# PufferAI/PufferLib

Hardware: AMD Instinct MI355X
Metric: env steps/sec end-to-end PPO (rollout+GAE+update), 4096 envs (higher is better)
Workload: dtype f32; 1 GPU; squared d=3 nt=1, 4096 envs/GPU x 128 steps, obs 49->64 f32 rows, MLP 128, 4 minibatches x 4 epochs, bptt 16 (BASELINE configs[1]); global_batch=524288, parallelism=dp1

## Files before the change

include/pufferlib_amd.h:

```cpp
#ifndef PUFFERLIB_AMD_H
#define PUFFERLIB_AMD_H
#include <stddef.h>
#include <stdint.h>

#ifdef __cplusplus
extern "C" {
#endif

typedef void *pfa_stream_t;

int pfa_version(void);
const char *pfa_last_error(void);

int pfa_timing_enable(int mode);
int pfa_timing_select(const char *kernel);
int pfa_timing_stride(int every);
int pfa_timing_reset(void);
int pfa_timing_read(const char *kernel, int64_t *launches_host, double *total_ms_host);

size_t pfa_gae_workspace_bytes(int64_t n);
int pfa_gae_f32(const float *dones, const float *values, const float *rewards, float *advantages,
                float *returns, int64_t n, float gamma, float gae_lambda, void *workspace,
                pfa_stream_t stream);
int pfa_gae_sums_supported(int64_t n, int32_t num_envs, int32_t num_minibatches, int32_t bptt_horizon);
size_t pfa_gae_sums_workspace_bytes(int64_t n, int32_t num_minibatches);
int pfa_gae_sums_f32(const float *dones, const float *values, const float *rewards, float *advantages, float *returns,
                     int64_t n, float gamma, float gae_lambda, int32_t num_envs, int32_t num_minibatches, int32_t bptt_horizon,
                     double *adv_stats, double *ev4, double *zero8, void *workspace, pfa_stream_t stream);
int32_t pfa_gae_halo_rows(float gamma, float gae_lambda);
int pfa_gae_halo_publish(const float *dones, const float *values, const float *rewards, int64_t n, float gamma, float gae_lambda,
                         const double *extra, int32_t n_extra, double *out, int32_t rank, int32_t world, pfa_stream_t stream);
int pfa_gae_halo_unpack(const double *gathered, int32_t rank, int32_t world, int64_t n, float gamma, float gae_lambda, float *dones,
                        float *values, float *rewards, pfa_stream_t stream);
int pfa_gae_halo_f32(const float *dones, const float *values, const float *rewards, float *advantages, float *returns, int64_t n,
                     int32_t halo_len, float gamma, float gae_lambda, int32_t num_envs, int32_t num_minibatches, int32_t bptt_horizon,
                     double *adv_stats, double *ev4, double *zero8, void *workspace, pfa_stream_t stream);
int pfa_gae_shard_pass2(const float *dones, const float *values, const float *rewards, float *advantages,
                        float *returns, int64_t n, int has_next, float gamma, float gae_lambda,
                        const void *workspace, const double *carry_in, pfa_stream_t stream);
int pfa_gae_shard_publish(const float *dones, const float *values, const float *rewards, int64_t n, float gamma, float gae_lambda,
                          void *workspace, const double *extra, int32_t n_extra, double *out, int32_t rank, int32_t world,
                          pfa_stream_t stream);
int pfa_gae_shard_fold(const double *gathered, int32_t rank, int32_t world, int64_t n, float gamma, float gae_lambda, void *workspace,
                       float *dones, float *values, float *rewards, double *carry_out, pfa_stream_t stream);


typedef struct {
    int32_t num_envs;
    int32_t distance_to_target;
    int32_t num_targets;
    int32_t obs_stride;
    int32_t tape_rounds;
} pfa_squared_config;

size_t pfa_squared_state_bytes(const pfa_squared_config *cfg);
int pfa_squared_async_reset(void *state, const pfa_squared_config *cfg, int64_t seed, float *obs,
                            float *rewards, uint8_t *terminals, uint8_t *truncations, uint8_t *masks,
                            pfa_stream_t stream);
int pfa_squared_fill_tape(void *state, const pfa_squared_config *cfg, int32_t rounds, pfa_stream_t stream);
int pfa_squared_send(void *state, const pfa_squared_config *cfg, const int64_t *actions, float *obs,
                     float *rewards, uint8_t *terminals, uint8_t *truncations, uint8_t *masks,
                     pfa_stream_t stream);
int pfa_squared_episode_stats(void *state, const pfa_squared_config *cfg, double *out4, int32_t reset,
                              pfa_stream_t stream);
int pfa_squared_last_infos(void *state, const pfa_squared_config *cfg, uint8_t *finished,
                           double *episode_return, int32_t *episode_length, double *score,
                           pfa_stream_t stream);
int pfa_squared_debug_targets(void *state, const pfa_squared_config *cfg, int32_t *cells, pfa_stream_t stream);
int pfa_squared_debug_stream_pos(void *state, const pfa_squared_config *cfg, uint64_t *pos_device, pfa_stream_t stream);

typedef struct {
    int32_t obs_dim;
    int32_t obs_stride;
    int32_t hidden;
    int32_t num_actions;
    uint32_t heads;
} pfa_mlp_dims;

int64_t pfa_mlp_param_count(const pfa_mlp_dims *dims);

typedef struct {
    uint64_t seed;
    uint64_t step;
} pfa_noise_key;

int pfa_mlp_forward_sample(const float *obs, int64_t rows, const float *params, const pfa_mlp_dims *dims,
                           const float *noise, const pfa_noise_key *key, int64_t row_offset,
                           int64_t *actions, float *logprob, float *entropy, float *value,
                           pfa_stream_t stream);

int pfa_philox_exp_noise(float *out, int64_t steps, int64_t rows, int32_t num_actions, const pfa_noise_key *key,
                         int64_t row_offset, pfa_stream_t stream);

typedef struct {
    float *obs;
    int32_t *actions;
    float *logprobs;
    float *values;
    float *rewards;
    float *dones;
    float *advantages;
    float *returns;
    int32_t horizon_T;
} pfa_experience;

int pfa_rollout_mlp_squared(void *state, const pfa_squared_config *cfg, const float *params,
                            const pfa_mlp_dims *dims, const pfa_experience *exp, const float *noise,
                            const pfa_noise_key *key, int64_t env_offset, float *obs, float *rewards,
                            uint8_t *terminals, uint8_t *truncations, uint8_t *masks, pfa_stream_t stream);

typedef struct pfa_mlp_view {
    const float *w1;
    int32_t ldw1, obs_dim, obs_stride, hidden, num_actions, reserved;
    const float *b1, *w2, *b2, *wv, *bv;
} pfa_mlp_view;
int pfa_mlp_view_supported(const pfa_mlp_view *view);
int pfa_mlp_view_forward_sample(const float *obs, int64_t rows, const pfa_mlp_view *view, const float *noise,
                                const pfa_noise_key *key, int64_t row_offset, int64_t *actions, float *logprob,
                                float *entropy, float *value, pfa_stream_t stream);
int pfa_rollout_mlp_view_squared(void *state, const pfa_squared_config *cfg, const pfa_mlp_view *view, const pfa_experience *exp,
                                 const float *noise, const pfa_noise_key *key, int64_t env_offset, float *obs, float *rewards,
                                 uint8_t *terminals, uint8_t *truncations, uint8_t *masks, pfa_stream_t stream);



size_t pfa_stochastic_state_bytes(int32_t num_envs);
int pfa_stochastic_async_reset(void *state, int32_t num_envs, float *obs, float *rewards, uint8_t *terminals,
                               uint8_t *truncations, uint8_t *masks, pfa_stream_t stream);
int pfa_stochastic_send(void *state, int32_t num_envs, double p, int32_t horizon, const int64_t *actions, float *obs,
                        float *rewards, uint8_t *terminals, uint8_t *truncations, uint8_t *masks, pfa_stream_t stream);
int pfa_stochastic_episode_stats(void *state, int32_t num_envs, double *out4, int32_t reset, pfa_stream_t stream);
int pfa_stochastic_last_infos(void *state, int32_t num_envs, uint8_t *finished, double *episode_return,
                              int32_t *episode_length, double *score, pfa_stream_t stream);
int pfa_rollout_mlp_stochastic(void *state, int32_t num_envs, double p, int32_t horizon, const float *params,
                               const pfa_mlp_dims *dims, const pfa_experience *exp, const float *noise,
                               const pfa_noise_key *key, int64_t env_offset, float *obs, float *rewards,
                               uint8_t *terminals, uint8_t *truncations, uint8_t *masks, pfa_stream_t stream);

typedef struct {
    int32_t num_envs;
    int32_t mem_length;
    int32_t mem_delay;
    int32_t tape_rounds;
} pfa_memory_config;
size_t pfa_memory_state_bytes(const pfa_memory_config *cfg);
int pfa_memory_async_reset(void *state, const pfa_memory_config *cfg, int64_t seed, float *obs, float *rewards,
                           uint8_t *terminals, uint8_t *truncations, uint8_t *masks, pfa_stream_t stream);
int pfa_memory_fill_tape(void *state, const pfa_memory_config *cfg, int32_t rounds, pfa_stream_t stream);
int pfa_memory_send(void *state, const pfa_memory_config *cfg, const int64_t *actions, float *obs, float *rewards,
                    uint8_t *terminals, uint8_t *truncations, uint8_t *masks, pfa_stream_t stream);
int pfa_memory_episode_stats(void *state, const pfa_memory_config *cfg, double *out4, int32_t reset, pfa_stream_t stream);
int pfa_memory_last_infos(void *state, const pfa_memory_config *cfg, uint8_t *finished, double *episode_return,
                          int32_t *episode_length, double *score, pfa_stream_t stream);
int pfa_memory_debug_solutions(void *state, const pfa_memory_config *cfg, uint32_t *bits, int32_t *underrun,
                               pfa_stream_t stream);

size_t pfa_bandit_state_bytes(int32_t num_envs);
int pfa_bandit_async_reset(void *state, int32_t num_envs, float *obs, float *rewards, uint8_t *terminals,
                           uint8_t *truncations, uint8_t *masks, pfa_stream_t stream);
int pfa_bandit_send(void *state, int32_t num_envs, int32_t solution, double reward_scale, const double *noise,
                    const int64_t *actions, float *obs, float *rewards, uint8_t *terminals, uint8_t *truncations,
                    uint8_t *masks, pfa_stream_t stream);
int pfa_bandit_episode_stats(void *state, int32_t num_envs, double *out4, int32_t reset, pfa_stream_t stream);
int pfa_bandit_last_infos(void *state, int32_t num_envs, uint8_t *finished, double *episode_return,
                          int32_t *episode_length, double *score, pfa_stream_t stream);

size_t pfa_multiagent_state_bytes(int32_t num_envs);
int pfa_multiagent_async_reset(void *state, int32_t num_envs, float *obs, float *rewards, uint8_t *terminals,
                               uint8_t *truncations, uint8_t *masks, pfa_stream_t stream);
int pfa_multiagent_send(void *state, int32_t num_envs, const int64_t *actions, float *obs, float *rewards,
                        uint8_t *terminals, uint8_t *truncations, uint8_t *masks, pfa_stream_t stream);
int pfa_multiagent_episode_stats(void *state, int32_t num_envs, double *out4, int32_t reset, pfa_stream_t stream);

typedef struct {
    int32_t num_envs;
    int32_t tape_rounds;
} pfa_spaces_config;
size_t pfa_spaces_state_bytes(const pfa_spaces_config *cfg);
int pfa_spaces_async_reset(void *state, const pfa_spaces_config *cfg, int64_t seed, float *obs, float *rewards,
                           uint8_t *terminals, uint8_t *truncations, uint8_t *masks, pfa_stream_t stream);
int pfa_spaces_fill_tape(void *state, const pfa_spaces_config *cfg, int32_t rounds, pfa_stream_t stream);
int pfa_spaces_send(void *state, const pfa_spaces_config *cfg, const int64_t *actions, float *obs, float *rewards,
                    uint8_t *terminals, uint8_t *truncations, uint8_t *masks, pfa_stream_t stream);
int pfa_spaces_episode_stats(void *state, const pfa_spaces_config *cfg, double *out5, int32_t reset, pfa_stream_t stream);
int pfa_spaces_last_infos(void *state, const pfa_spaces_config *cfg, uint8_t *finished, double *episode_return,
                          int32_t *episode_length, double *score, pfa_stream_t stream);

typedef struct {
    int32_t num_envs;
    int32_t obs_values;
    int32_t obs_stride;
    int32_t num_actions;
    int32_t episode_length;
    int32_t obs_high;
    uint64_t seed;
    int64_t env_offset;
} pfa_synth_config;
size_t pfa_synth_state_bytes(const pfa_synth_config *cfg);
int pfa_synth_async_reset(void *state, const pfa_synth_config *cfg, float *obs, float *rewards, uint8_t *terminals,
                          uint8_t *truncations, uint8_t *masks, pfa_stream_t stream);
int pfa_synth_send(void *state, const pfa_synth_config *cfg, const int64_t *actions, float *obs, float *rewards,
                   uint8_t *terminals, uint8_t *truncations, uint8_t *masks, pfa_stream_t stream);
int pfa_frames_async_reset(void *state, const pfa_synth_config *cfg, uint8_t *obs, float *rewards, uint8_t *terminals,
                           uint8_t *truncations, uint8_t *masks, pfa_stream_t stream);
int pfa_frames_send(void *state, const pfa_synth_config *cfg, const int64_t *actions, uint8_t *obs, float *rewards,
                    uint8_t *terminals, uint8_t *truncations, uint8_t *masks, pfa_stream_t stream);
int pfa_synth_episode_stats(void *state, const pfa_synth_config *cfg, double *out4, int32_t reset, pfa_stream_t stream);
int pfa_synth_last_infos(void *state, const pfa_synth_config *cfg, uint8_t *finished, double *episode_return,
                         int32_t *episode_length, double *score, pfa_stream_t stream);

#define PFA_NAT_MAX_FIELDS 32
typedef enum {
    PFA_NAT_U8 = 0, PFA_NAT_I8 = 1, PFA_NAT_U16 = 2, PFA_NAT_I16 = 3, PFA_NAT_U32 = 4, PFA_NAT_I32 = 5,
    PFA_NAT_U64 = 6, PFA_NAT_I64 = 7, PFA_NAT_F16 = 8, PFA_NAT_F32 = 9, PFA_NAT_F64 = 10
} pfa_nat_dtype;
typedef struct {
    void *out;
    int32_t offset;
    int32_t count;
    int32_t dtype;
    int32_t to_f32;
    int32_t out_stride;
    int32_t reserved;
} pfa_nat_field;
int pfa_nativize_rows(const void *rows, int64_t num_rows, int32_t row_bytes, const pfa_nat_field *fields ,
                      int32_t num_fields, pfa_stream_t stream);

typedef struct {
    float clip_coef, vf_clip_coef, vf_coef, ent_coef;
    int32_t norm_adv, clip_vloss;
    int32_t num_minibatches;
    int32_t bptt_horizon;
} pfa_ppo_hparams;

size_t pfa_ppo_workspace_bytes(const pfa_mlp_dims *dims, int64_t batch_rows, const pfa_ppo_hparams *hp);
int pfa_ppo_adv_stats(const pfa_experience *exp, int64_t batch_rows, const pfa_ppo_hparams *hp,
                      double *stats, void *workspace, pfa_stream_t stream);
int pfa_ppo_mlp_grad(const pfa_experience *exp, int64_t batch_rows, int32_t mb, const float *params,
                     const pfa_mlp_dims *dims, const pfa_ppo_hparams *hp, const double *adv_stats,
                     int64_t global_mb_rows, float *grads, void *workspace, pfa_stream_t stream);
int pfa_ppo_mlp_grad_mfma_per_tile(int32_t obs_dim, int32_t obs_stride, int32_t num_actions);
int pfa_ppo_grid_status(void);
int pfa_ppo_grid_reset(void);
int pfa_ppo_mlp_grad_path(const pfa_mlp_dims *dims, int64_t mb_rows);
int pfa_adam_clip_step(float *params, const float *grads, float *exp_avg, float *exp_avg_sq, int64_t count,
                       float lr, float beta1, float beta2, float eps, int64_t step, float max_grad_norm,
                       float grad_scale, const float *loss_sums, double *losses, double loss_scale,
                       const double *norm_partials, int32_t n_norm_partials, pfa_stream_t stream);

int pfa_ppo_mlp_train(const pfa_experience *exp, int64_t batch_rows, float *params, const pfa_mlp_dims *dims,
                      const pfa_ppo_hparams *hp, const double *adv_stats, float *grads, float *exp_avg,
                      float *exp_avg_sq, int64_t opt_step, float lr, float beta1, float beta2, float eps,
                      float max_grad_norm, int32_t update_epochs, double *losses, void *workspace,
                      int32_t data_parallel, pfa_stream_t stream);
int pfa_ppo_mlp_train_logged(const pfa_experience *exp, int64_t batch_rows, float *params, const pfa_mlp_dims *dims,
                             const pfa_ppo_hparams *hp, const double *adv_stats, float *grads, float *exp_avg,
                             float *exp_avg_sq, int64_t opt_step, float lr, float beta1, float beta2, float eps,
                             float max_grad_norm, int32_t update_epochs, double *losses, void *workspace,
                             int32_t data_parallel, const double *log_ev4, double *log_out10, int32_t *log_packed,
                             pfa_stream_t stream);

int pfa_ppo_wide_supported(const pfa_mlp_view *view);
size_t pfa_ppo_wide_workspace_bytes(const pfa_mlp_view *view);
int pfa_ppo_wide_grad(const pfa_experience *exp, int64_t batch_rows, int32_t mb, const pfa_mlp_view *params, const pfa_mlp_view *grads,
                      float *tail16, const pfa_ppo_hparams *hp, const double *adv_stats, int64_t global_mb_rows, void *workspace,
                      pfa_stream_t stream);

int64_t pfa_lstm_param_count(const pfa_mlp_dims *dims);
size_t pfa_lstm_pack_bytes(void);
int pfa_lstm_pack(const float *params, const pfa_mlp_dims *dims, void *wpack, pfa_stream_t stream);
int pfa_lstm_policy_step(const float *obs, int64_t rows, const float *params, const pfa_mlp_dims *dims,
                         const void *wpack, float *h, float *c, const float *noise, const pfa_noise_key *key,
                         int64_t row_offset, int64_t *actions, float *logprob, float *entropy, float *value,
                         pfa_stream_t stream);
int pfa_rollout_lstm_squared(void *state, const pfa_squared_config *cfg, const float *params,
                             const pfa_mlp_dims *dims, const void *wpack, float *h, float *c,
                             const pfa_experience *exp, const float *noise, const pfa_noise_key *key,
                             int64_t env_offset, float *obs, float *rewards, uint8_t *terminals,
                             uint8_t *truncations, uint8_t *masks, pfa_stream_t stream);
int pfa_rollout_lstm_memory(void *state, const pfa_memory_config *cfg, const float *params, const pfa_mlp_dims *dims,
                            const void *wpack, float *h, float *c, const pfa_experience *exp, const float *noise,
                            const pfa_noise_key *key, int64_t env_offset, float *obs, float *rewards, uint8_t *terminals,
                            uint8_t *truncations, uint8_t *masks, pfa_stream_t stream);
int pfa_rollout_lstm_synth(void *state, const pfa_synth_config *cfg, const float *params, const pfa_mlp_dims *dims,
                           const void *wpack, float *h, float *c, const pfa_experience *exp, const float *noise,
                           const pfa_noise_key *key, int64_t env_offset, float *obs, float *rewards, uint8_t *terminals,
                           uint8_t *truncations, uint8_t *masks, pfa_stream_t stream);
int pfa_lstm_pack_bwd(const float *params, const pfa_mlp_dims *dims, void *wpack_bwd, pfa_stream_t stream);
int pfa_lstm_pack_both(const float *params, const pfa_mlp_dims *dims, void *wpack, void *wpack_bwd, pfa_stream_t stream);
int pfa_lstm_seq_forward(const float *obs_tm, int64_t rows, int32_t steps, const float *params, const pfa_mlp_dims *dims,
                         const void *wpack, float *xe, float *gates_act, float *hs, float *cs, int32_t init_slot, pfa_stream_t stream);
size_t pfa_lstm_seq_backward_workspace_bytes(int64_t rows);
int pfa_lstm_seq_backward(const float *gates_act, const float *cs, const float *xe, const float *dh_heads, int64_t rows,
                          int32_t steps, const void *wpack_bwd, float *dgates, float *dxe, float *gate_bias_grad,
                          float *enc_bias_grad, void *workspace, pfa_stream_t stream);
int pfa_store_step(const pfa_experience *exp, int32_t t, int32_t num_envs, int32_t obs_stride, const float *obs,
                   const float *rewards, const uint8_t *terminals, const int64_t *actions, const float *logprob,
                   const float *value, pfa_stream_t stream);
int pfa_store_rows(const pfa_experience *exp, int32_t rows, int32_t num_slots, int32_t obs_stride, const float *obs,
                   const float *rewards, const uint8_t *dones, const int64_t *actions, const float *logprob,
                   const float *value, const int32_t *env_ids, const uint8_t *mask, int32_t *counters,
                   int32_t *stored_dropped, pfa_stream_t stream);
int pfa_store_rows_bytes(const pfa_experience *exp, int32_t rows, int32_t num_slots, int32_t row_bytes, const uint8_t *obs,
                         const float *rewards, const uint8_t *dones, const int64_t *actions, const float *logprob,
                         const float *value, const int32_t *env_ids, const uint8_t *mask, int32_t *counters,
                         int32_t *stored_dropped, pfa_stream_t stream);
int pfa_gather_obs_time_major(const pfa_experience *exp, int64_t batch_rows, int32_t mb, const pfa_ppo_hparams *hp,
                              int32_t obs_stride, float *out, pfa_stream_t stream);
size_t pfa_lstm_heads_loss_workspace_bytes(void);
int pfa_lstm_heads_loss(const float *h, const pfa_experience *exp, int64_t batch_rows, int32_t mb, const float *params,
                        const pfa_mlp_dims *dims, const pfa_ppo_hparams *hp, const double *adv_stats,
                        int64_t global_mb_rows, float *dout, float *dh, float *loss_sums8, float *head_bias_grad16,
                        void *workspace, pfa_stream_t stream);
size_t pfa_gemm_tn_workspace_bytes(int32_t mo, int32_t no, int64_t k);
int pfa_gemm_tn_f32(const float *a, int64_t lda, const float *b, int64_t ldb, float *c, int64_t ldc, int32_t mo,
                    int32_t no, int64_t k, void *workspace, pfa_stream_t stream);
size_t pfa_gemm_tn2_workspace_bytes(int32_t mo, int64_t k);
typedef struct pfa_reduce_job {
    int32_t kind, splits, mo, no;
    const float *partial;
    float *c;
    int64_t ldc;
    float *c2;
    int64_t ldc2;
    int32_t nb, reserved;
} pfa_reduce_job;
int pfa_gemm_tn_partial_f32(const float *a, int64_t lda, const float *b, int64_t ldb, int32_t mo, int32_t no, int64_t k, void *workspace,
                            pfa_reduce_job *job, pfa_stream_t stream);
int pfa_gemm_tn2_partial_f32(const float *a, int64_t lda, const float *b0, int64_t ldb0, const float *b1, int64_t ldb1, int32_t mo, int64_t k,
                             void *workspace, pfa_reduce_job *job, pfa_stream_t stream);
int pfa_reduce_multi(const pfa_reduce_job *jobs, int32_t njobs, pfa_stream_t stream);
int pfa_gemm_tn2_f32(const float *a, int64_t lda, const float *b0, int64_t ldb0, const float *b1, int64_t ldb1, float *c0, int64_t ldc0,
                     float *c1, int64_t ldc1, int32_t mo, int64_t k, void *workspace, pfa_stream_t stream);
int pfa_lstm_finish_grads(float *grads, const pfa_mlp_dims *dims, const float *g16, const float *bsum16, pfa_stream_t stream);
int pfa_sumsq_partials(const float *grads, int64_t count, double *partials, int32_t n, pfa_stream_t stream);

int pfa_dist_unique_id(uint8_t *id128_host);
int pfa_dist_init(const uint8_t *id128_host, int32_t rank, int32_t world);
int pfa_dist_finalize(void);
int pfa_dist_all_reduce_f32(float *buf, int64_t count, pfa_stream_t stream);
int pfa_dist_all_reduce_f64(double *buf, int64_t count, pfa_stream_t stream);
int pfa_dist_info(int64_t *out8);

typedef struct {
    int32_t mode;
    int32_t reserved;
    const void *ptr;
    int64_t lda;
    int32_t IC, IH, IW, OC, OH, OW, KH, KW, S;
    int32_t sc, sy, sx, frame_bytes;
} pfa_igemm_operand;
int pfa_igemm_rows(const pfa_igemm_operand *a, int64_t M, int32_t K, const float *B, int32_t ldb, int32_t N, float *C, int32_t ldc,
                   int32_t epilogue, const float *bias, const float *mask, int32_t ldmask, pfa_stream_t stream);
int pfa_igemm_set_products(int32_t mode);
int pfa_igemm_get_products(void);
size_t pfa_igemm_weights_workspace_bytes(int64_t M, int32_t K, int32_t N);
int pfa_igemm_weights(const pfa_igemm_operand *a, int64_t M, int32_t K, const float *D, int32_t ldd, int32_t N, float *out,
                      int32_t perm, int32_t accumulate, float *bias_out, void *workspace, pfa_stream_t stream);
size_t pfa_colsum_workspace_bytes(int32_t N);
int pfa_colsum(const float *D, int64_t M, int32_t N, int32_t ldd, float *out, int32_t accumulate, void *workspace, pfa_stream_t stream);
int pfa_cnn_pack_conv(const float *w, const pfa_igemm_operand *geom, int32_t u8_order, float *fwd, float *dx, pfa_stream_t stream);
int pfa_igemm_rows_add(const pfa_igemm_operand *a, int64_t M, int32_t K, const float *B, int32_t ldb, int32_t N, float *C, int32_t ldc,
                       int32_t epilogue, const float *bias, const float *mask, int32_t ldmask, const float *addend, int32_t ldadd,
                       pfa_stream_t stream);
int pfa_cnn_pack_conv_same(const float *w, const pfa_igemm_operand *geom, int32_t u8, float *fwd, int32_t ldf, float *dx, pfa_stream_t stream);
int pfa_maxpool3s2_forward(const float *in, int64_t frames, int32_t H, int32_t W, int32_t channels, float *out, pfa_stream_t stream);
int pfa_maxpool3s2_backward(const float *in, const float *out, const float *dout, int64_t frames, int32_t H, int32_t W, int32_t channels,
                            float *din, pfa_stream_t stream);
int pfa_cnn_transpose(const float *w, int32_t N, int32_t K, float *out, pfa_stream_t stream);
int pfa_cnn_pack_fc(const float *w, int32_t N, int32_t channels, int32_t hw, float *perm_out, float *t_out, pfa_stream_t stream);
int pfa_cnn_heads_sample(const float *h, int64_t rows, const float *actor_w, const float *actor_b, const float *value_w,
                         const float *value_b, int32_t num_actions, const float *noise, const pfa_noise_key *key, int64_t row_offset,
                         int64_t *actions, float *logprob, float *entropy, float *value, pfa_stream_t stream);
int pfa_cnn_heads_sample_w(const float *h, int32_t hidden, int64_t rows, const float *actor_w, const float *actor_b, const float *value_w,
                           const float *value_b, int32_t num_actions, const float *noise, const pfa_noise_key *key, int64_t row_offset,
                           int64_t *actions, float *logprob, float *entropy, float *value, pfa_stream_t stream);
size_t pfa_cnn_heads_loss_workspace_bytes(void);
int pfa_cnn_heads_loss(const float *h, const pfa_experience *exp, int64_t batch_rows, int32_t mb, int64_t q0, int64_t rows,
                       const float *actor_w, const float *actor_b, const float *value_w, const float *value_b, int32_t num_actions,
                       const pfa_ppo_hparams *hp, const double *adv_stats, int64_t global_mb_rows, float *dout, float *dh,
                       float *loss_pairs16, int32_t accumulate, void *workspace, pfa_stream_t stream);
int pfa_cnn_heads_loss_w(const float *h, int32_t hidden, const pfa_experience *exp, int64_t batch_rows, int32_t mb, int64_t q0, int64_t rows,
                         const float *actor_w, const float *actor_b, const float *value_w, const float *value_b, int32_t num_actions,
                         const pfa_ppo_hparams *hp, const double *adv_stats, int64_t global_mb_rows, float *dout, float *dh,
                         float *loss_pairs16, int32_t accumulate, void *workspace, pfa_stream_t stream);
int pfa_cnn_gather_frames(const uint8_t *frames, int64_t frame_bytes, int64_t batch_rows, int32_t mb, const pfa_ppo_hparams *hp,
                          int64_t q0, int64_t rows, uint8_t *out, pfa_stream_t stream);

int pfa_heads_rows_sample(const float *out, int32_t ld, int64_t rows, int32_t num_actions, uint32_t heads, const float *noise,
                          const pfa_noise_key *key, int64_t row_offset, int64_t *actions, float *logprob, float *entropy,
                          float *value, pfa_stream_t stream);
int pfa_heads_rows_eval(const float *out, int32_t ld, int64_t rows, int32_t num_actions, uint32_t heads, const int64_t *actions,
                        float *logprob, float *entropy, float *value, pfa_stream_t stream);
size_t pfa_heads_rows_loss_workspace_bytes(int64_t rows);
int pfa_heads_rows_loss(const float *out, int32_t ld, const pfa_experience *exp, int64_t batch_rows, int32_t mb, int64_t q0,
                        int64_t rows, int32_t time_major_rows, int32_t num_actions, uint32_t heads, const pfa_ppo_hparams *hp,
                        const double *adv_stats, int64_t global_mb_rows, float *dout, int32_t ldd, int32_t num_out,
                        float *loss_pairs16, int32_t accumulate, void *workspace, pfa_stream_t stream);
int pfa_lstm_cell_forward(float *gates, const float *c_prev, float *c_out, float *h_out, int32_t ldh, float *h_out2, int32_t ldh2,
                          int64_t rows, int32_t hidden, pfa_stream_t stream);
int pfa_lstm_cell_backward(const float *dh_a, int32_t lda, const float *dh_b, int32_t ldb, float *dc, const float *gates_act,
                           const float *c_prev, const float *c, float *dgates, int64_t rows, int32_t hidden, pfa_stream_t stream);
int pfa_rows_perm(const float *src, int32_t lds_, float *dst, int32_t ldd, const float *act, int32_t lda, int64_t rows, int32_t cols,
                  int32_t segments, int32_t steps, int32_t to_time_major, pfa_stream_t stream);

int pfa_p2p_alloc(int64_t cap_bytes, int32_t world, uint8_t *handle64_host);
int pfa_p2p_open(const uint8_t *handles_host, int32_t rank, int32_t world);
int pfa_p2p_close(void);
int pfa_p2p_status(void);
int64_t pfa_p2p_seq(void);
int pfa_p2p_reset(int64_t base);
int pfa_p2p_debug_set_status(int value);
int pfa_p2p_all_reduce_f32(float *buf, int64_t count, pfa_stream_t stream);
int pfa_p2p_all_reduce_f64(double *buf, int64_t count, pfa_stream_t stream);
int pfa_p2p_ll_all_reduce_f32(float *buf, int64_t count, pfa_stream_t stream);
int64_t pfa_p2p_ll_calls(void);
int pfa_p2p_wait_stats(int64_t *out4_host, int reset);
int pfa_p2p_enable(int on);

int pfa_train_log_sums(const pfa_experience *exp, int64_t batch_rows, int32_t num_envs, const double *losses,
                       double *out10, void *workspace, pfa_stream_t stream);

int pfa_train_ev_sums(const pfa_experience *exp, int64_t batch_rows, int32_t num_envs, double *out4, void *workspace,
                      pfa_stream_t stream);
int pfa_train_log_pack(const double *losses, const double *ev4, double *out10, pfa_stream_t stream);

#ifdef __cplusplus
}
#endif
#endif
```

pufferlib_amd/_lib.py:

```python
import ctypes as C
import os
import subprocess

from .exceptions import ExtensionError

HERE = os.path.dirname(os.path.abspath(__file__))
REPO = os.path.dirname(HERE)
CSRC = os.path.join(HERE, 'csrc')
LIB_DIR = os.path.join(HERE, '_lib')
LIB_PATH = os.path.join(LIB_DIR, 'libpufferlib_amd.so')
SOURCES = ['common.cpp', 'dist.cpp', 'p2p.hip', 'gae.hip', 'squared.hip', 'rollout.hip', 'ppo_update.hip', 'lstm.hip', 'gemm.hip', 'lstm_fused.hip', 'lstm_seq.hip', 'stochastic.hip', 'memory.hip', 'bandit.hip', 'multiagent.hip', 'spaces.hip', 'synthetic.hip', 'nativize.hip', 'igemm.hip', 'cnn_heads.hip', 'general.hip', 'ppo_wide.hip']
HEADERS = sorted(f for f in os.listdir(CSRC) if f.endswith('.hpp')) + [os.path.join('..', '..', 'include', 'pufferlib_amd.h')]


def _stale():
    if not os.path.exists(LIB_PATH):
        return True
    t = os.path.getmtime(LIB_PATH)
    deps = [os.path.join(CSRC, f) for f in SOURCES + HEADERS]
    return any(os.path.exists(d) and os.path.getmtime(d) > t for d in deps)


def source_hash():
    import hashlib
    h = hashlib.sha256()
    for f in SOURCES + HEADERS:
        with open(os.path.join(CSRC, f), 'rb') as fh:
            h.update(fh.read())
    return h.hexdigest()[:16]


def build(force=False, verbose=False):
    if not force and not _stale():
        return LIB_PATH
    os.makedirs(LIB_DIR, exist_ok=True)
    hipcc = os.environ.get('HIPCC', '/opt/rocm/bin/hipcc')
    objs = []
    procs = []
    import shlex
    extra = shlex.split(os.environ.get('PFA_HIPCC_FLAGS', ''))
    for src in SOURCES:
        obj = os.path.join(LIB_DIR, os.path.splitext(src)[0] + '.o')
        objs.append(obj)
        cmd = [hipcc, '--offload-arch=gfx950', '-O3', '-std=c++17', '-fPIC'] + extra + ['-x', 'hip', '-c',
               os.path.join(CSRC, src), '-o', obj]
        if verbose:
            print(' '.join(cmd))
        procs.append((src, subprocess.Popen(cmd, stdout=subprocess.PIPE, stderr=subprocess.STDOUT)))
    for src, p in procs:
        out, _ = p.communicate()
        if p.returncode != 0:
            raise ExtensionError(f'hipcc failed on {src}:\n{out.decode()}')
    cmd = [hipcc, '--offload-arch=gfx950', '-shared', '-fPIC', '-o', LIB_PATH] + objs + ['-ldl']
    r = subprocess.run(cmd, stdout=subprocess.PIPE, stderr=subprocess.STDOUT)
    if r.returncode != 0:
        raise ExtensionError(f'link failed:\n{r.stdout.decode()}')
    return LIB_PATH


class SquaredConfig(C.Structure):
    _fields_ = [('num_envs', C.c_int32), ('distance_to_target', C.c_int32), ('num_targets', C.c_int32),
                ('obs_stride', C.c_int32), ('tape_rounds', C.c_int32)]


NAT_MAX_FIELDS = 32


class NatField(C.Structure):
    _fields_ = [('out', C.c_void_p), ('offset', C.c_int32), ('count', C.c_int32), ('dtype', C.c_int32), ('to_f32', C.c_int32),
                ('out_stride', C.c_int32), ('reserved', C.c_int32)]


class MemoryConfig(C.Structure):
    _fields_ = [('num_envs', C.c_int32), ('mem_length', C.c_int32), ('mem_delay', C.c_int32), ('tape_rounds', C.c_int32)]


class SpacesConfig(C.Structure):
    _fields_ = [('num_envs', C.c_int32), ('tape_rounds', C.c_int32)]


class SynthConfig(C.Structure):
    _fields_ = [('num_envs', C.c_int32), ('obs_values', C.c_int32), ('obs_stride', C.c_int32), ('num_actions', C.c_int32),
                ('episode_length', C.c_int32), ('obs_high', C.c_int32), ('seed', C.c_uint64), ('env_offset', C.c_int64)]


class IgemmOperand(C.Structure):
    _fields_ = [('mode', C.c_int32), ('reserved', C.c_int32), ('ptr', C.c_void_p), ('lda', C.c_int64), ('IC', C.c_int32), ('IH', C.c_int32),
                ('IW', C.c_int32), ('OC', C.c_int32), ('OH', C.c_int32), ('OW', C.c_int32), ('KH', C.c_int32), ('KW', C.c_int32), ('S', C.c_int32),
                ('sc', C.c_int32), ('sy', C.c_int32), ('sx', C.c_int32), ('frame_bytes', C.c_int32)]


class MlpDims(C.Structure):
    _fields_ = [('obs_dim', C.c_int32), ('obs_stride', C.c_int32), ('hidden', C.c_int32), ('num_actions', C.c_int32),
                ('heads', C.c_uint32)]


class MlpView(C.Structure):
    _fields_ = [('w1', C.c_void_p), ('ldw1', C.c_int32), ('obs_dim', C.c_int32), ('obs_stride', C.c_int32), ('hidden', C.c_int32),
                ('num_actions', C.c_int32), ('reserved', C.c_int32), ('b1', C.c_void_p), ('w2', C.c_void_p), ('b2', C.c_void_p),
                ('wv', C.c_void_p), ('bv', C.c_void_p)]


class NoiseKey(C.Structure):
    _fields_ = [('seed', C.c_uint64), ('step', C.c_uint64)]


class Experience(C.Structure):
    _fields_ = [('obs', C.c_void_p), ('actions', C.c_void_p), ('logprobs', C.c_void_p), ('values', C.c_void_p),
                ('rewards', C.c_void_p), ('dones', C.c_void_p), ('advantages', C.c_void_p), ('returns', C.c_void_p),
                ('horizon_T', C.c_int32)]


class ReduceJob(C.Structure):
    _fields_ = [('kind', C.c_int32), ('splits', C.c_int32), ('mo', C.c_int32), ('no', C.c_int32), ('partial', C.c_void_p), ('c', C.c_void_p),
                ('ldc', C.c_int64), ('c2', C.c_void_p), ('ldc2', C.c_int64), ('nb', C.c_int32), ('reserved', C.c_int32)]


class PpoHparams(C.Structure):
    _fields_ = [('clip_coef', C.c_float), ('vf_clip_coef', C.c_float), ('vf_coef', C.c_float), ('ent_coef', C.c_float),
                ('norm_adv', C.c_int32), ('clip_vloss', C.c_int32), ('num_minibatches', C.c_int32),
                ('bptt_horizon', C.c_int32)]


P = C.c_void_p
_SIGNATURES = {
    'pfa_version': (C.c_int, []),
    'pfa_last_error': (C.c_char_p, []),
    'pfa_timing_enable': (C.c_int, [C.c_int]),
    'pfa_timing_select': (C.c_int, [C.c_char_p]),
    'pfa_timing_stride': (C.c_int, [C.c_int]),
    'pfa_timing_reset': (C.c_int, []),
    'pfa_timing_read': (C.c_int, [C.c_char_p, C.POINTER(C.c_int64), C.POINTER(C.c_double)]),
    'pfa_gae_workspace_bytes': (C.c_size_t, [C.c_int64]),
    'pfa_gae_f32': (C.c_int, [P, P, P, P, P, C.c_int64, C.c_float, C.c_float, P, P]),
    'pfa_gae_sums_supported': (C.c_int, [C.c_int64, C.c_int32, C.c_int32, C.c_int32]),
    'pfa_gae_sums_workspace_bytes': (C.c_size_t, [C.c_int64, C.c_int32]),
    'pfa_gae_sums_f32': (C.c_int, [P, P, P, P, P, C.c_int64, C.c_float, C.c_float, C.c_int32, C.c_int32, C.c_int32, P, P, P, P, P]),
    'pfa_gae_halo_rows': (C.c_int32, [C.c_float, C.c_float]),
    'pfa_gae_halo_publish': (C.c_int, [P, P, P, C.c_int64, C.c_float, C.c_float, P, C.c_int32, P, C.c_int32, C.c_int32, P]),
    'pfa_gae_halo_unpack': (C.c_int, [P, C.c_int32, C.c_int32, C.c_int64, C.c_float, C.c_float, P, P, P, P]),
    'pfa_gae_halo_f32': (C.c_int, [P, P, P, P, P, C.c_int64, C.c_int32, C.c_float, C.c_float, C.c_int32, C.c_int32, C.c_int32, P, P, P, P, P]),
    'pfa_gae_shard_pass2': (C.c_int, [P, P, P, P, P, C.c_int64, C.c_int, C.c_float, C.c_float, P, P, P]),
    'pfa_gae_shard_publish': (C.c_int, [P, P, P, C.c_int64, C.c_float, C.c_float, P, P, C.c_int32, P, C.c_int32, C.c_int32, P]),
    'pfa_gae_shard_fold': (C.c_int, [P, C.c_int32, C.c_int32, C.c_int64, C.c_float, C.c_float, P, P, P, P, P, P]),
    'pfa_train_ev_sums': (C.c_int, [C.POINTER(Experience), C.c_int64, C.c_int32, P, P, P]),
    'pfa_train_log_pack': (C.c_int, [P, P, P, P]),
    'pfa_squared_state_bytes': (C.c_size_t, [C.POINTER(SquaredConfig)]),
    'pfa_squared_async_reset': (C.c_int, [P, C.POINTER(SquaredConfig), C.c_int64, P, P, P, P, P, P]),
    'pfa_squared_fill_tape': (C.c_int, [P, C.POINTER(SquaredConfig), C.c_int32, P]),
    'pfa_squared_send': (C.c_int, [P, C.POINTER(SquaredConfig), P, P, P, P, P, P, P]),
    'pfa_squared_episode_stats': (C.c_int, [P, C.POINTER(SquaredConfig), P, C.c_int32, P]),
    'pfa_squared_last_infos': (C.c_int, [P, C.POINTER(SquaredConfig), P, P, P, P, P]),
    'pfa_squared_debug_targets': (C.c_int, [P, C.POINTER(SquaredConfig), P, P]),
    'pfa_squared_debug_stream_pos': (C.c_int, [P, C.POINTER(SquaredConfig), P, P]),
    'pfa_mlp_param_count': (C.c_int64, [C.POINTER(MlpDims)]),
    'pfa_mlp_forward_sample': (C.c_int, [P, C.c_int64, P, C.POINTER(MlpDims), P, C.POINTER(NoiseKey), C.c_int64,
                                         P, P, P, P, P]),
    'pfa_philox_exp_noise': (C.c_int, [P, C.c_int64, C.c_int64, C.c_int32, C.POINTER(NoiseKey), C.c_int64, P]),
    'pfa_rollout_mlp_squared': (C.c_int, [P, C.POINTER(SquaredConfig), P, C.POINTER(MlpDims), C.POINTER(Experience),
                                          P, C.POINTER(NoiseKey), C.c_int64, P, P, P, P, P, P]),
    'pfa_mlp_view_supported': (C.c_int, [C.POINTER(MlpView)]),
    'pfa_ppo_wide_supported': (C.c_int, [C.POINTER(MlpView)]),
    'pfa_ppo_wide_workspace_bytes': (C.c_size_t, [C.POINTER(MlpView)]),
    'pfa_ppo_wide_grad': (C.c_int, [C.POINTER(Experience), C.c_int64, C.c_int32, C.POINTER(MlpView), C.POINTER(MlpView), P, C.POINTER(PpoHparams), P,
                                    C.c_int64, P, P]),
    'pfa_mlp_view_forward_sample': (C.c_int, [P, C.c_int64, C.POINTER(MlpView), P, C.POINTER(NoiseKey), C.c_int64, P, P, P, P, P]),
    'pfa_rollout_mlp_view_squared': (C.c_int, [P, C.POINTER(SquaredConfig), C.POINTER(MlpView), C.POINTER(Experience), P, C.POINTER(NoiseKey),
                                               C.c_int64, P, P, P, P, P, P]),
    'pfa_stochastic_state_bytes': (C.c_size_t, [C.c_int32]),
    'pfa_stochastic_async_reset': (C.c_int, [P, C.c_int32, P, P, P, P, P, P]),
    'pfa_stochastic_send': (C.c_int, [P, C.c_int32, C.c_double, C.c_int32, P, P, P, P, P, P, P]),
    'pfa_stochastic_episode_stats': (C.c_int, [P, C.c_int32, P, C.c_int32, P]),
    'pfa_stochastic_last_infos': (C.c_int, [P, C.c_int32, P, P, P, P, P]),
    'pfa_rollout_mlp_stochastic': (C.c_int, [P, C.c_int32, C.c_double, C.c_int32, P, C.POINTER(MlpDims), C.POINTER(Experience),
                                             P, C.POINTER(NoiseKey), C.c_int64, P, P, P, P, P, P]),
    'pfa_memory_state_bytes': (C.c_size_t, [C.POINTER(MemoryConfig)]),
    'pfa_memory_async_reset': (C.c_int, [P, C.POINTER(MemoryConfig), C.c_int64, P, P, P, P, P, P]),
    'pfa_memory_fill_tape': (C.c_int, [P, C.POINTER(MemoryConfig), C.c_int32, P]),
    'pfa_memory_send': (C.c_int, [P, C.POINTER(MemoryConfig), P, P, P, P, P, P, P]),
    'pfa_memory_episode_stats': (C.c_int, [P, C.POINTER(MemoryConfig), P, C.c_int32, P]),
    'pfa_memory_last_infos': (C.c_int, [P, C.POINTER(MemoryConfig), P, P, P, P, P]),
    'pfa_memory_debug_solutions': (C.c_int, [P, C.POINTER(MemoryConfig), P, P, P]),
    'pfa_bandit_state_bytes': (C.c_size_t, [C.c_int32]),
    'pfa_bandit_async_reset': (C.c_int, [P, C.c_int32, P, P, P, P, P, P]),
    'pfa_bandit_send': (C.c_int, [P, C.c_int32, C.c_int32, C.c_double, P, P, P, P, P, P, P, P]),
    'pfa_bandit_episode_stats': (C.c_int, [P, C.c_int32, P, C.c_int32, P]),
    'pfa_bandit_last_infos': (C.c_int, [P, C.c_int32, P, P, P, P, P]),
    'pfa_multiagent_state_bytes': (C.c_size_t, [C.c_int32]),
    'pfa_multiagent_async_reset': (C.c_int, [P, C.c_int32, P, P, P, P, P, P]),
    'pfa_multiagent_send': (C.c_int, [P, C.c_int32, P, P, P, P, P, P, P]),
    'pfa_spaces_state_bytes': (C.c_size_t, [C.POINTER(SpacesConfig)]),
    'pfa_spaces_async_reset': (C.c_int, [P, C.POINTER(SpacesConfig), C.c_int64, P, P, P, P, P, P]),
    'pfa_spaces_fill_tape': (C.c_int, [P, C.POINTER(SpacesConfig), C.c_int32, P]),
    'pfa_spaces_send': (C.c_int, [P, C.POINTER(SpacesConfig), P, P, P, P, P, P, P]),
    'pfa_spaces_episode_stats': (C.c_int, [P, C.POINTER(SpacesConfig), P, C.c_int32, P]),
    'pfa_spaces_last_infos': (C.c_int, [P, C.POINTER(SpacesConfig), P, P, P, P, P]),
    'pfa_synth_state_bytes': (C.c_size_t, [C.POINTER(SynthConfig)]),
    'pfa_synth_async_reset': (C.c_int, [P, C.POINTER(SynthConfig), P, P, P, P, P, P]),
    'pfa_synth_send': (C.c_int, [P, C.POINTER(SynthConfig), P, P, P, P, P, P, P]),
    'pfa_frames_async_reset': (C.c_int, [P, C.POINTER(SynthConfig), P, P, P, P, P, P]),
    'pfa_frames_send': (C.c_int, [P, C.POINTER(SynthConfig), P, P, P, P, P, P, P]),
    'pfa_synth_episode_stats': (C.c_int, [P, C.POINTER(SynthConfig), P, C.c_int32, P]),
    'pfa_synth_last_infos': (C.c_int, [P, C.POINTER(SynthConfig), P, P, P, P, P]),
    'pfa_multiagent_episode_stats': (C.c_int, [P, C.c_int32, P, C.c_int32, P]),
    'pfa_nativize_rows': (C.c_int, [P, C.c_int64, C.c_int32, P, C.c_int32, P]),
    'pfa_ppo_workspace_bytes': (C.c_size_t, [C.POINTER(MlpDims), C.c_int64, C.POINTER(PpoHparams)]),
    'pfa_ppo_adv_stats': (C.c_int, [C.POINTER(Experience), C.c_int64, C.POINTER(PpoHparams), P, P, P]),
    'pfa_ppo_mlp_grad': (C.c_int, [C.POINTER(Experience), C.c_int64, C.c_int32, P, C.POINTER(MlpDims),
                                   C.POINTER(PpoHparams), P, C.c_int64, P, P, P]),
    'pfa_ppo_mlp_train': (C.c_int, [C.POINTER(Experience), C.c_int64, P, C.POINTER(MlpDims), C.POINTER(PpoHparams), P, P, P, P,
                                    C.c_int64, C.c_float, C.c_float, C.c_float, C.c_float, C.c_float, C.c_int32, P, P,
                                    C.c_int32, P]),
    'pfa_ppo_mlp_train_logged': (C.c_int, [C.POINTER(Experience), C.c_int64, P, C.POINTER(MlpDims), C.POINTER(PpoHparams), P, P, P, P,
                                           C.c_int64, C.c_float, C.c_float, C.c_float, C.c_float, C.c_float, C.c_int32, P, P,
                                           C.c_int32, P, P, C.POINTER(C.c_int32), P]),
    'pfa_store_step': (C.c_int, [C.POINTER(Experience), C.c_int32, C.c_int32, C.c_int32, P, P, P, P, P, P, P]),
    'pfa_store_rows': (C.c_int, [C.POINTER(Experience), C.c_int32, C.c_int32, C.c_int32, P, P, P, P, P, P, P, P, P, P, P]),
    'pfa_store_rows_bytes': (C.c_int, [C.POINTER(Experience), C.c_int32, C.c_int32, C.c_int32, P, P, P, P, P, P, P, P, P, P, P]),
    'pfa_gather_obs_time_major': (C.c_int, [C.POINTER(Experience), C.c_int64, C.c_int32, C.POINTER(PpoHparams), C.c_int32, P, P]),
    'pfa_lstm_heads_loss_workspace_bytes': (C.c_size_t, []),
    'pfa_lstm_heads_loss': (C.c_int, [P, C.POINTER(Experience), C.c_int64, C.c_int32, P, C.POINTER(MlpDims),
                                      C.POINTER(PpoHparams), P, C.c_int64, P, P, P, P, P, P]),
    'pfa_lstm_param_count': (C.c_int64, [C.POINTER(MlpDims)]),
    'pfa_lstm_pack_bytes': (C.c_size_t, []),
    'pfa_lstm_pack': (C.c_int, [P, C.POINTER(MlpDims), P, P]),
    'pfa_lstm_policy_step': (C.c_int, [P, C.c_int64, P, C.POINTER(MlpDims), P, P, P, P, C.POINTER(NoiseKey), C.c_int64,
                                       P, P, P, P, P]),
    'pfa_rollout_lstm_squared': (C.c_int, [P, C.POINTER(SquaredConfig), P, C.POINTER(MlpDims), P, P, P, C.POINTER(Experience),
                                           P, C.POINTER(NoiseKey), C.c_int64, P, P, P, P, P, P]),
    'pfa_rollout_lstm_memory': (C.c_int, [P, C.POINTER(MemoryConfig), P, C.POINTER(MlpDims), P, P, P, C.POINTER(Experience),
                                           P, C.POINTER(NoiseKey), C.c_int64, P, P, P, P, P, P]),
    'pfa_rollout_lstm_synth': (C.c_int, [P, C.POINTER(SynthConfig), P, C.POINTER(MlpDims), P, P, P, C.POINTER(Experience),
                                           P, C.POINTER(NoiseKey), C.c_int64, P, P, P, P, P, P]),
    'pfa_lstm_pack_bwd': (C.c_int, [P, C.POINTER(MlpDims), P, P]),
    'pfa_lstm_seq_forward': (C.c_int, [P, C.c_int64, C.c_int32, P, C.POINTER(MlpDims), P, P, P, P, P, C.c_int32, P]),
    'pfa_lstm_pack_both': (C.c_int, [P, C.POINTER(MlpDims), P, P, P]),
    'pfa_lstm_seq_backward_workspace_bytes': (C.c_size_t, [C.c_int64]),
    'pfa_lstm_seq_backward': (C.c_int, [P, P, P, P, C.c_int64, C.c_int32, P, P, P, P, P, P, P]),
    'pfa_gemm_tn_workspace_bytes': (C.c_size_t, [C.c_int32, C.c_int32, C.c_int64]),
    'pfa_gemm_tn_f32': (C.c_int, [P, C.c_int64, P, C.c_int64, P, C.c_int64, C.c_int32, C.c_int32, C.c_int64, P, P]),
    'pfa_gemm_tn2_workspace_bytes': (C.c_size_t, [C.c_int32, C.c_int64]),
    'pfa_gemm_tn_partial_f32': (C.c_int, [P, C.c_int64, P, C.c_int64, C.c_int32, C.c_int32, C.c_int64, P, C.POINTER(ReduceJob), P]),
    'pfa_gemm_tn2_partial_f32': (C.c_int, [P, C.c_int64, P, C.c_int64, P, C.c_int64, C.c_int32, C.c_int64, P, C.POINTER(ReduceJob), P]),
    'pfa_reduce_multi': (C.c_int, [C.POINTER(ReduceJob), C.c_int32, P]),
    'pfa_gemm_tn2_f32': (C.c_int, [P, C.c_int64, P, C.c_int64, P, C.c_int64, P, C.c_int64, P, C.c_int64, C.c_int32, C.c_int64, P, P]),
    'pfa_lstm_finish_grads': (C.c_int, [P, C.POINTER(MlpDims), P, P, P]),
    'pfa_sumsq_partials': (C.c_int, [P, C.c_int64, P, C.c_int32, P]),
    'pfa_dist_unique_id': (C.c_int, [P]),
    'pfa_dist_init': (C.c_int, [P, C.c_int32, C.c_int32]),
    'pfa_dist_finalize': (C.c_int, []),
    'pfa_dist_all_reduce_f32': (C.c_int, [P, C.c_int64, P]),
    'pfa_dist_all_reduce_f64': (C.c_int, [P, C.c_int64, P]),
    'pfa_dist_info': (C.c_int, [P]),
    'pfa_ppo_mlp_grad_mfma_per_tile': (C.c_int, [C.c_int32, C.c_int32, C.c_int32]),
    'pfa_ppo_mlp_grad_path': (C.c_int, [C.POINTER(MlpDims), C.c_int64]),
    'pfa_heads_rows_sample': (C.c_int, [P, C.c_int32, C.c_int64, C.c_int32, C.c_uint32, P, C.POINTER(NoiseKey), C.c_int64, P, P, P, P, P]),
    'pfa_heads_rows_eval': (C.c_int, [P, C.c_int32, C.c_int64, C.c_int32, C.c_uint32, P, P, P, P, P]),
    'pfa_heads_rows_loss_workspace_bytes': (C.c_size_t, [C.c_int64]),
    'pfa_heads_rows_loss': (C.c_int, [P, C.c_int32, C.POINTER(Experience), C.c_int64, C.c_int32, C.c_int64, C.c_int64, C.c_int32, C.c_int32,
                                      C.c_uint32, C.POINTER(PpoHparams), P, C.c_int64, P, C.c_int32, C.c_int32, P, C.c_int32, P, P]),
    'pfa_lstm_cell_forward': (C.c_int, [P, P, P, P, C.c_int32, P, C.c_int32, C.c_int64, C.c_int32, P]),
    'pfa_lstm_cell_backward': (C.c_int, [P, C.c_int32, P, C.c_int32, P, P, P, P, P, C.c_int64, C.c_int32, P]),
    'pfa_rows_perm': (C.c_int, [P, C.c_int32, P, C.c_int32, P, C.c_int32, C.c_int64, C.c_int32, C.c_int32, C.c_int32, C.c_int32, P]),
    'pfa_igemm_set_products': (C.c_int, [C.c_int32]),
    'pfa_igemm_get_products': (C.c_int, []),
    'pfa_igemm_rows': (C.c_int, [C.POINTER(IgemmOperand), C.c_int64, C.c_int32, P, C.c_int32, C.c_int32, P, C.c_int32, C.c_int32, P, P, C.c_int32, P]),
    'pfa_igemm_weights_workspace_bytes': (C.c_size_t, [C.c_int64, C.c_int32, C.c_int32]),
    'pfa_igemm_weights': (C.c_int, [C.POINTER(IgemmOperand), C.c_int64, C.c_int32, P, C.c_int32, C.c_int32, P, C.c_int32, C.c_int32, P, P, P]),
    'pfa_colsum_workspace_bytes': (C.c_size_t, [C.c_int32]),
    'pfa_colsum': (C.c_int, [P, C.c_int64, C.c_int32, C.c_int32, P, C.c_int32, P, P]),
    'pfa_cnn_pack_conv': (C.c_int, [P, C.POINTER(IgemmOperand), C.c_int32, P, P, P]),
    'pfa_igemm_rows_add': (C.c_int, [C.POINTER(IgemmOperand), C.c_int64, C.c_int32, P, C.c_int32, C.c_int32, P, C.c_int32, C.c_int32, P, P, C.c_int32, P,
                                     C.c_int32, P]),
    'pfa_cnn_pack_conv_same': (C.c_int, [P, C.POINTER(IgemmOperand), C.c_int32, P, C.c_int32, P, P]),
    'pfa_maxpool3s2_forward': (C.c_int, [P, C.c_int64, C.c_int32, C.c_int32, C.c_int32, P, P]),
    'pfa_maxpool3s2_backward': (C.c_int, [P, P, P, C.c_int64, C.c_int32, C.c_int32, C.c_int32, P, P]),
    'pfa_cnn_transpose': (C.c_int, [P, C.c_int32, C.c_int32, P, P]),
    'pfa_cnn_pack_fc': (C.c_int, [P, C.c_int32, C.c_int32, C.c_int32, P, P, P]),
    'pfa_cnn_heads_sample': (C.c_int, [P, C.c_int64, P, P, P, P, C.c_int32, P, C.POINTER(NoiseKey), C.c_int64, P, P, P, P, P]),
    'pfa_cnn_heads_sample_w': (C.c_int, [P, C.c_int32, C.c_int64, P, P, P, P, C.c_int32, P, C.POINTER(NoiseKey), C.c_int64, P, P, P, P, P]),
    'pfa_cnn_heads_loss_w': (C.c_int, [P, C.c_int32, C.POINTER(Experience), C.c_int64, C.c_int32, C.c_int64, C.c_int64, P, P, P, P, C.c_int32,
                                       C.POINTER(PpoHparams), P, C.c_int64, P, P, P, C.c_int32, P, P]),
    'pfa_cnn_heads_loss_workspace_bytes': (C.c_size_t, []),
    'pfa_cnn_heads_loss': (C.c_int, [P, C.POINTER(Experience), C.c_int64, C.c_int32, C.c_int64, C.c_int64, P, P, P, P, C.c_int32,
                                     C.POINTER(PpoHparams), P, C.c_int64, P, P, P, C.c_int32, P, P]),
    'pfa_cnn_gather_frames': (C.c_int, [P, C.c_int64, C.c_int64, C.c_int32, C.POINTER(PpoHparams), C.c_int64, C.c_int64, P, P]),
    'pfa_p2p_alloc': (C.c_int, [C.c_int64, C.c_int32, P]),
    'pfa_p2p_open': (C.c_int, [P, C.c_int32, C.c_int32]),
    'pfa_p2p_close': (C.c_int, []),
    'pfa_p2p_status': (C.c_int, []),
    'pfa_ppo_grid_status': (C.c_int, []),
    'pfa_ppo_grid_reset': (C.c_int, []),
    'pfa_p2p_seq': (C.c_int64, []),
    'pfa_p2p_reset': (C.c_int, [C.c_int64]),
    'pfa_p2p_debug_set_status': (C.c_int, [C.c_int]),
    'pfa_p2p_all_reduce_f32': (C.c_int, [P, C.c_int64, P]),
    'pfa_p2p_all_reduce_f64': (C.c_int, [P, C.c_int64, P]),
    'pfa_p2p_ll_all_reduce_f32': (C.c_int, [P, C.c_int64, P]),
    'pfa_p2p_ll_calls': (C.c_int64, []),
    'pfa_p2p_wait_stats': (C.c_int, [P, C.c_int]),
    'pfa_p2p_enable': (C.c_int, [C.c_int]),
    'pfa_train_log_sums': (C.c_int, [C.POINTER(Experience), C.c_int64, C.c_int32, P, P, P, P]),
    'pfa_adam_clip_step': (C.c_int, [P, P, P, P, C.c_int64, C.c_float, C.c_float, C.c_float, C.c_float, C.c_int64,
                                     C.c_float, C.c_float, P, P, C.c_double, P, C.c_int32, P]),
}

_lib = None


def lib():
    global _lib
    if _lib is not None:
        return _lib
    if not os.path.exists(LIB_PATH):
        raise ExtensionError(
            f'{LIB_PATH} is missing: run `python -c "import __graft_entry__ as g; g.build()"` '
            '(hipcc --offload-arch=gfx950).  pufferlib_amd has no CPU fallback.')
    import torch
    try:
        L = C.CDLL(LIB_PATH)
    except OSError as e:
        raise ExtensionError(f'cannot load {LIB_PATH}: {e}') from e
    for name, (res, args) in _SIGNATURES.items():
        try:
            f = getattr(L, name)
        except AttributeError as e:
            raise ExtensionError(f'{LIB_PATH} does not export {name}') from e
        f.restype = res
        f.argtypes = args
    _lib = L
    form = os.environ.get('PFA_MATRIX_PRODUCTS', 'fp32')
    if form not in ('fp32', 'bf16x6'):
        raise ExtensionError(f"PFA_MATRIX_PRODUCTS={form!r}: expected 'fp32' or 'bf16x6'")
    if form == 'bf16x6':
        check(L.pfa_igemm_set_products(1), 'PFA_MATRIX_PRODUCTS')
    return L


def check(rc, what=''):
    if rc != 0:
        msg = lib().pfa_last_error().decode(errors='replace')
        raise ExtensionError(f'{what} failed ({rc}): {msg}')


def ptr(t):
    return None if t is None else C.c_void_p(t.data_ptr())


def stream_handle():
    import torch
    return C.c_void_p(torch.cuda.current_stream().cuda_stream)


def require_gpu():
    import torch
    if not torch.cuda.is_available():
        raise ExtensionError('pufferlib_amd needs a ROCm GPU (torch.cuda.is_available() is False); '
                             'there is no CPU fallback')
```

pufferlib_amd/csrc/ppo_tile.hpp:

```cpp
#pragma once
#include <cmath>

#ifndef PFA_LOSS_EXP_REPAIR_ALL
#define PFA_LOSS_EXP_REPAIR_ALL 0
#endif

#include "common.hpp"
#include "mlp_tile.hpp"

namespace pfa {

constexpr int kNumStats = 8;

struct RowMap {
    int mb, nmb, horizon;
    __device__ __forceinline__ long long flat(long long q) const {
        const long long k = q / horizon, h = q - k * horizon;
        return ((long long)mb + k * nmb) * horizon + h;
    }
    __device__ __forceinline__ unsigned row32(unsigned q) const {
        const unsigned k = q / (unsigned)horizon, h = q - k * (unsigned)horizon;
        return ((unsigned)mb + k * (unsigned)nmb) * (unsigned)horizon + h;
    }
    __device__ __forceinline__ unsigned tile_first(unsigned tile) const {
        return row32(__builtin_amdgcn_readfirstlane(tile) * 16u);
    }
    __device__ __forceinline__ unsigned tile_row(unsigned tile, unsigned first, int r, bool aligned) const {
        return aligned ? first + (unsigned)r : row32(tile * 16u + (unsigned)r);
    }
};

__device__ __forceinline__ void wave_lds_fence() {
    __builtin_amdgcn_fence(__ATOMIC_RELEASE, "wavefront");
    __builtin_amdgcn_wave_barrier();
}

template <bool SWAP>
__device__ __forceinline__ float gsum(float x) {
    if constexpr (SWAP) {
        auto p = __builtin_amdgcn_permlane16_swap(__float_as_uint(x), __float_as_uint(x), false, false);
        const float s = __uint_as_float(p[0]) + __uint_as_float(p[1]);
        auto q = __builtin_amdgcn_permlane32_swap(__float_as_uint(s), __float_as_uint(s), false, false);
        return __uint_as_float(q[0]) + __uint_as_float(q[1]);
    } else {
        x += __shfl_xor(x, 16, 64);
        x += __shfl_xor(x, 32, 64);
        return x;
    }
}
template <bool SWAP>
__device__ __forceinline__ float gmax(float x) {
    if constexpr (SWAP) {
        auto p = __builtin_amdgcn_permlane16_swap(__float_as_uint(x), __float_as_uint(x), false, false);
        const float s = fmaxf(__uint_as_float(p[0]), __uint_as_float(p[1]));
        auto q = __builtin_amdgcn_permlane32_swap(__float_as_uint(s), __float_as_uint(s), false, false);
        return fmaxf(__uint_as_float(q[0]), __uint_as_float(q[1]));
    } else {
        x = fmaxf(x, __shfl_xor(x, 16, 64));
        x = fmaxf(x, __shfl_xor(x, 32, 64));
        return x;
    }
}

__device__ __forceinline__ float loss_exp(float x) {
    const float kL = 1.44269502162933349609375f, kLl = 1.92596298909109e-8f;
    const float t = x * kL;
    const float e = fmaf(x, kLl, fmaf(x, kL, -t));
    const float r = __builtin_amdgcn_exp2f(t);
    return fmaf(r, e * 0.693147182464599609375f, r);
}
__device__ __forceinline__ float loss_exp_softmax(float x) {
#if PFA_LOSS_EXP_REPAIR_ALL
    return loss_exp(x);
#else
    return __builtin_amdgcn_exp2f(x * 1.44269502162933349609375f);
#endif
}
__device__ __forceinline__ float loss_log(float x) {
    const float l2 = __builtin_amdgcn_logf(x);
    return fmaf(l2, 0.693147182464599609375f, l2 * -1.904654323148236e-9f);
}

struct RowScalars {
    int action;
    float old_logprob, old_value, adv, ret, weight;
};

struct LossOut {
    f32x4 dout;
    float pg, v_loss, ent, neg_logratio, kl, clipped;
};

template <bool MH, bool SWAP = false, bool PERM = false>
__device__ __forceinline__ LossOut ppo_loss_tile(const f32x4 &out, const RowScalars &rs, int a, uint32_t heads, int g,
                                                 const pfa_ppo_hparams &hp, float adv_mean, float adv_rden, float inv_rows) {
    float nl[4], p[4], hent[4], ent = 0.0f, new_logprob = 0.0f, new_value = 0.0f;
    bool chosen[4];
    if constexpr (MH) {
#pragma unroll
        for (int r = 0; r < 4; ++r) {
            nl[r] = p[r] = hent[r] = 0.0f;
            chosen[r] = false;
            if (4 * g + r == a) new_value = out[r];
        }
        int start = 0;
        for (int h = 0; h < 8; ++h) {
            const int sz = (int)((heads >> (4 * h)) & 15u);
            if (sz == 0) break;
            bool mem[4];
            float lmax = -INFINITY;
#pragma unroll
            for (int r = 0; r < 4; ++r) {
                const int o = 4 * g + r;
                mem[r] = o >= start && o < start + sz;
                if (mem[r]) lmax = fmaxf(lmax, out[r]);
            }
            lmax = fmaxf(lmax, __shfl_xor(lmax, 16, 64));
            lmax = fmaxf(lmax, __shfl_xor(lmax, 32, 64));
            float ev[4], se = 0.0f;
#pragma unroll
            for (int r = 0; r < 4; ++r) {
                ev[r] = mem[r] ? loss_exp(out[r] - lmax) : 0.0f;
                se += ev[r];
            }
            se += __shfl_xor(se, 16, 64);
            se += __shfl_xor(se, 32, 64);
            const float lse = lmax + loss_log(se), inv_se = __builtin_amdgcn_rcpf(se);
            const int act = start + (int)(((uint32_t)rs.action >> (4 * h)) & 15u);
            float he = 0.0f;
#pragma unroll
            for (int r = 0; r < 4; ++r)
                if (mem[r]) {
                    nl[r] = out[r] - lse;
                    p[r] = ev[r] * inv_se;
                    he -= nl[r] * p[r];
                    chosen[r] = 4 * g + r == act;
                    if (chosen[r]) new_logprob += nl[r];
                }
            he += __shfl_xor(he, 16, 64);
            he += __shfl_xor(he, 32, 64);
#pragma unroll
            for (int r = 0; r < 4; ++r)
                if (mem[r]) hent[r] = he;
            ent += he;
            start += sz;
        }
        new_logprob += __shfl_xor(new_logprob, 16, 64);
        new_logprob += __shfl_xor(new_logprob, 32, 64);
        new_value += __shfl_xor(new_value, 16, 64);
        new_value += __shfl_xor(new_value, 32, 64);
    } else {
    static_assert(!(MH && PERM), "the permuted layout is the single-head form");
    constexpr int NR = PERM ? 3 : 4;
    const int o0 = PERM ? 3 * g : 4 * g;
#pragma unroll
    for (int r = NR; r < 4; ++r) {
        nl[r] = p[r] = 0.0f;
        chosen[r] = false;
    }
    float lmax = -INFINITY;
#pragma unroll
    for (int r = 0; r < NR; ++r)
        if (o0 + r < a) lmax = fmaxf(lmax, out[r]);
    lmax = gmax<SWAP>(lmax);
    float ev[4], se = 0.0f;
#pragma unroll
    for (int r = 0; r < NR; ++r) {
        ev[r] = o0 + r < a ? loss_exp_softmax(out[r] - lmax) : 0.0f;
        se += ev[r];
    }
    se = gsum<SWAP>(se);
    const float lse = lmax + loss_log(se);
    const float inv_se = __builtin_amdgcn_rcpf(se);
#pragma unroll
    for (int r = 0; r < NR; ++r) {
        const int o = o0 + r;
        nl[r] = out[r] - lse;
        p[r] = ev[r] * inv_se;
        if (o < a) ent -= nl[r] * p[r];
        chosen[r] = o == rs.action;
        if (chosen[r]) new_logprob = nl[r];
        if (o == a) new_value = out[r];
    }
    ent = gsum<SWAP>(ent);
    new_logprob = gsum<SWAP>(new_logprob);
    new_value = gsum<SWAP>(new_value);
#pragma unroll
    for (int r = 0; r < 4; ++r) hent[r] = ent;
    }

    const float logratio = new_logprob - rs.old_logprob;
    const float ratio = loss_exp(logratio);
    const float adv = hp.norm_adv ? (rs.adv - adv_mean) * adv_rden : rs.adv;
    const float lo = 1.0f - hp.clip_coef, hi = 1.0f + hp.clip_coef;
    const float pg1 = -adv * ratio;
    const float pg2 = -adv * fminf(fmaxf(ratio, lo), hi);
    const bool inside = ratio >= lo && ratio <= hi;
    float dpg_dratio;
    if (pg1 > pg2) dpg_dratio = -adv;
    else if (pg1 < pg2) dpg_dratio = inside ? -adv : 0.0f;
    else dpg_dratio = inside ? -adv : -0.5f * adv;
    const float scale = inv_rows * rs.weight;
    const float g_lp = dpg_dratio * ratio * scale;

    float v_loss, dv;
    if (hp.clip_vloss) {
        const float du = new_value - rs.ret;
        const float vl_u = du * du;
        const float delta = new_value - rs.old_value;
        const float v_clipped = rs.old_value + fminf(fmaxf(delta, -hp.vf_clip_coef), hp.vf_clip_coef);
        const float dc = v_clipped - rs.ret;
        const float vl_c = dc * dc;
        const bool vin = delta >= -hp.vf_clip_coef && delta <= hp.vf_clip_coef;
        v_loss = 0.5f * fmaxf(vl_u, vl_c);
        const float gu = 2.0f * du, gc = vin ? 2.0f * dc : 0.0f;
        const float sel = vl_u > vl_c ? gu : (vl_u < vl_c ? gc : 0.5f * (gu + gc));
        dv = 0.5f * sel;
    } else {
        const float du = new_value - rs.ret;
        v_loss = 0.5f * du * du;
        dv = du;
    }
    dv *= hp.vf_coef * scale;

    LossOut lo_;
#pragma unroll
    for (int r = 0; r < 4; ++r) {
        const int o = PERM ? (r < 3 ? 3 * g + r : 99) : 4 * g + r;
        float d = 0.0f;
        if (o < a) {
            d = g_lp * ((chosen[r] ? 1.0f : 0.0f) - p[r]) + hp.ent_coef * scale * p[r] * (nl[r] + hent[r]);
        } else if (o == a) {
            d = dv;
        }
        lo_.dout[r] = d;
    }
    lo_.pg = fmaxf(pg1, pg2) * rs.weight;
    lo_.v_loss = v_loss * rs.weight;
    lo_.ent = ent * rs.weight;
    lo_.neg_logratio = -logratio * rs.weight;
    lo_.kl = ((ratio - 1.0f) - logratio) * rs.weight;
    lo_.clipped = (fabsf(ratio - 1.0f) > hp.clip_coef ? 1.0f : 0.0f) * rs.weight;
    return lo_;
}

constexpr int kTailFloats = 2 * kNumStats;


}
```

pufferlib_amd/csrc/ppo_update.hip:

```cpp
#include <cmath>
#include <cstdlib>
#include <type_traits>

#include <hip/hip_ext.h>

#include <unordered_map>

#include "common.hpp"
#include "mlp_tile.hpp"
#include "sampler.hpp"
#include "ppo_tile.hpp"
#include "p2p_ll.hpp"

#ifndef PFA_GRAD_FCOL
#define PFA_GRAD_FCOL 1
#endif
#ifndef PFA_GRAD_GLDS
#define PFA_GRAD_GLDS 0
#endif
#ifndef PFA_GRAD_PIPE
#define PFA_GRAD_PIPE 1
#endif

namespace pfa {

constexpr int grad_pairs(int dp) { return dp <= 64 ? 4 : 2; }
constexpr int grad_threads(int dp) { return grad_pairs(dp) * 2 * 64; }
constexpr int grad_waves_per_simd(int dp) { return dp <= 64 ? 2 : 1; }

constexpr bool grad_glds(int dp, int ktm) { return PFA_GRAD_GLDS && PFA_GRAD_PIPE && dp == 64 && ktm <= 3; }
template <int DP, bool GL = false>
struct GradLds {
    static constexpr int XS = XTile<DP>::XS;
    static constexpr int KS = DP / 4;
    static constexpr int W1S = KS + 4;
    static constexpr int HS = kHidden + 4;
    static constexpr int DS = 20;
    static constexpr int kXSlot = GL ? 16 * DP : 16 * XS;
    static constexpr int kXSlots = GL ? 3 : 2;
    static constexpr int kXT = 0;
    static constexpr int kHT = kXSlots * kXSlot;
    static constexpr int kDT = kHT + 16 * HS;
    static constexpr int kPairFloats = kDT + 16 * DS;
    static constexpr int kW1Floats = kMT * 64 * W1S;
    static constexpr int kTabFloats = kMT * 64 * 4;
    static constexpr int kFloats = grad_pairs(DP) * kPairFloats + kW1Floats + 3 * kTabFloats;
    __device__ static __forceinline__ int xi(int row, int col) {
        if constexpr (GL) {
            const int kk = col >> 2;
            return (kk >> 2) * 256 + (((kk & 3) << 4) + (row & 12) + ((row + kk) & 3)) * 4 + (col & 3);
        } else {
            return row * XS + col;
        }
    }
};

template <int DP, int KTM = DP / 16, bool COL = false>
struct NativeLayout {
    static constexpr int kDw1 = 0;
    static constexpr int kCol = kDw1 + KTM * kMT * 4 * 64;
    static constexpr int kDw2 = kCol + (COL ? kHidden : 0);
    static constexpr int kDb1 = kDw2 + kMT * 4 * 64;
    static constexpr int kDb2 = kDb1 + kHidden;
    static constexpr int kStats = kDb2 + kOut;
    static constexpr int kCount = kStats + kNumStats;
};

}
#include "ppo_bf16.hpp"
namespace pfa {

#ifdef PFA_PROBES
__device__ unsigned long long *g_trace = nullptr;
__device__ int g_trace_tiles = 0;
#define PFA_STAMP(j, k)                                                                                         \
    do {                                                                                                        \
        if (g_trace && blockIdx.x == 0 && lane == 0 && (j) < g_trace_tiles)                                     \
            g_trace[((size_t)wv * g_trace_tiles + (j)) * 8 + (k)] = __builtin_amdgcn_s_memtime();               \
    } while (0)
#else
#define PFA_STAMP(j, k) do { } while (0)
#endif

__host__ __device__ constexpr int slot_output(bool perm, int slot) {
    return !perm ? slot : ((slot & 3) == 3 ? 99 : 3 * (slot >> 2) + (slot & 3));
}
template <int DP, int ABL = 0, int KKU = DP / 4, bool MH = false, int KTM = DP / 16, bool COL = false, bool PERM = false>
__global__ void __launch_bounds__(grad_threads(DP), grad_waves_per_simd(DP))
    ppo_mlp_grad_kernel(pfa_experience ex, RowMap map, long long mb_rows, const float *params, int a, uint32_t heads,
                        pfa_ppo_hparams hp, const double *adv_stats , double global_rows, float *partials) {
    constexpr bool kGlds = grad_glds(DP, KTM);
    using L = GradLds<DP, kGlds>;
    using NL = NativeLayout<DP, KTM, COL>;
    constexpr int XS = L::XS, HS = L::HS, DS = L::DS, KS = DP / 4, V = DP / 4, W1S = L::W1S;
    constexpr int NLD = (16 * V + 63) / 64;
    constexpr int kGradPairs = grad_pairs(DP), kGradThreads = grad_threads(DP);
    constexpr bool kQuad = kGradPairs == 4 && 4 * NL::kCount <= L::kFloats;
    constexpr bool kPipe = PFA_GRAD_PIPE && (DP <= 32 || (DP == 64 && KTM <= 3));
    constexpr bool FCOL = PFA_GRAD_FCOL && COL && kPipe && KKU > 4 * KTM;
    constexpr int KKM = FCOL ? 4 * KTM : KKU;
    static_assert(!PERM || (kPipe && !MH), "the permuted head layout is wired into the pipelined single-head form");
    extern __shared__ __attribute__((aligned(16))) float lds[];
    const int lane = lane_id(), wv = wave_id(), c = lane & 15, g = lane >> 4;
    const int pair = wv & (kGradPairs - 1);
    const bool producer = wv < kGradPairs;
    float *pl = lds + pair * L::kPairFloats;
    float *w1t = lds + kGradPairs * L::kPairFloats;
    float *b1t = w1t + L::kW1Floats;
    float *w2t = b1t + L::kTabFloats;
    float *w2bt = w2t + L::kTabFloats;
    const MlpOffsets off = mlp_offsets(DP, a);

#ifndef PFA_DBG_SKIP_TABLES
    {
        constexpr int N1 = kMT * 64 * KS / kGradThreads, N2 = kMT * 64 * 4 / kGradThreads;
        static_assert(kMT * 64 * KS % kGradThreads == 0 && kMT * 64 * 4 % kGradThreads == 0, "table sizes");
        constexpr int CH = N1 > 16 ? 16 : N1;
        static_assert(N1 % CH == 0, "table chunking");
        float tb[N2], tw[N2], tv[N2];
#pragma unroll
        for (int j = 0; j < N2; ++j) {
            const int i = threadIdx.x + j * kGradThreads;
            const int r = i & 3, ln = (i >> 2) & 63, m = i >> 8, cc = ln & 15, gg = ln >> 4;
            tb[j] = params[off.b1 + 16 * m + 4 * gg + r];
            tw[j] = w2v_at(params, off, a, slot_output(PERM, cc), 16 * m + 4 * gg + r);
            tv[j] = w2v_at(params, off, a, slot_output(PERM, 4 * gg + r), 16 * m + cc);
        }
#pragma unroll 1
        for (int j0 = 0; j0 < N1; j0 += CH) {
            float t1[CH];
#pragma unroll
            for (int j = 0; j < CH; ++j) {
                const int i = threadIdx.x + (j0 + j) * kGradThreads;
                const int kk = i % KS, ln = (i / KS) & 63, m = i / (KS * 64), cc = ln & 15, gg = ln >> 4;
                t1[j] = params[off.w1 + (16 * m + cc) * DP + 4 * kk + gg];
            }
#pragma unroll
            for (int j = 0; j < CH; ++j) {
                const int i = threadIdx.x + (j0 + j) * kGradThreads;
                const int kk = i % KS, ln = (i / KS) & 63, m = i / (KS * 64);
                w1t[(m * 64 + ln) * W1S + kk] = t1[j];
            }
        }
#pragma unroll
        for (int j = 0; j < N2; ++j) {
            const int i = threadIdx.x + j * kGradThreads;
            b1t[i] = tb[j];
            w2t[i] = tw[j];
            w2bt[i] = tv[j];
        }
        if constexpr (FCOL) {
            static_assert(W1S - KS >= 4 && KS % 4 == 0, "the trailing-column fragment sits in the lane's pad floats");
            float tc[N2];
#pragma unroll
            for (int j = 0; j < N2; ++j) {
                const int i = threadIdx.x + j * kGradThreads;
                const int r = i & 3, ln = (i >> 2) & 63, m = i >> 8, gg = ln >> 4;
                tc[j] = params[off.w1 + (16 * m + 4 * gg + r) * DP + 16 * KTM];
            }
#pragma unroll
            for (int j = 0; j < N2; ++j) {
                const int i = threadIdx.x + j * kGradThreads;
                w1t[(i >> 2) * W1S + KS + (i & 3)] = tc[j];
            }
        }
    }
#endif

    const long long tiles = mb_rows / 16;
    const long long pair_global = (long long)blockIdx.x * kGradPairs + pair;
    const long long pair_count = (long long)gridDim.x * kGradPairs;
    const int J = (int)((tiles + pair_count - 1) / pair_count);
    const bool aligned = (map.horizon & 15) == 0;

    if (producer) {
        float bo[4];
#pragma unroll
        for (int r = 0; r < 4; ++r) bo[r] = b2v_at(params, off, a, slot_output(PERM, 4 * g + r));
        float adv_mean = 0.0f, adv_den = 1.0f;
        if (hp.norm_adv) {
            const double s1 = adv_stats[2 * map.mb], s2 = adv_stats[2 * map.mb + 1];
            const double mean = s1 / global_rows;
            double var = (s2 - s1 * mean) / (global_rows - 1.0);
            var = var > 0.0 ? var : 0.0;
            adv_mean = (float)mean;
            adv_den = (float)sqrt(var) + 1e-8f;
        }
        const float inv_rows = (float)(1.0 / global_rows);
        const float adv_rden = 1.0f / adv_den;

        f32x4 acc_dw2[kMT];
        float db2[4], stats[6];
#pragma unroll
        for (int m = 0; m < kMT; ++m) acc_dw2[m] = f32x4{0.f, 0.f, 0.f, 0.f};
#pragma unroll
        for (int r = 0; r < 4; ++r) db2[r] = 0.0f;
#pragma unroll
        for (int i = 0; i < 6; ++i) stats[i] = 0.0f;

        float4 xpre[kGlds ? 1 : NLD];
        RowScalars rspre;
        auto prefetch = [&](long long tile, float *xdst) {
            const bool ok = tile < tiles;
            const unsigned first = ok ? map.tile_first((unsigned)tile) : 0u;
            rspre = RowScalars{0, 0.f, 0.f, 0.f, 0.f, 0.f};
            if (ok) {
                const unsigned fr = map.tile_row((unsigned)tile, first, c, aligned);
                rspre = RowScalars{ex.actions[fr], ex.logprobs[fr], ex.values[fr], ex.advantages[fr], ex.returns[fr], 1.0f};
            }
            if constexpr (kGlds) {
                const int kl = lane >> 4, row = (lane & 12) + ((lane - kl) & 3);
                if (ok) {
                    const unsigned frow = map.tile_row((unsigned)tile, first, row, aligned);
                    const float *src = ex.obs + (size_t)frow * DP + 4 * kl;
#pragma unroll
                    for (int b = 0; b < DP / 16; ++b)
                        __builtin_amdgcn_global_load_lds(src + 16 * b, (__attribute__((address_space(3))) void *)(xdst + 256 * b), 16, 0, 0);
                } else {
#pragma unroll
                    for (int b = 0; b < DP / 16; ++b) *reinterpret_cast<float4 *>(xdst + 256 * b + 4 * lane) = make_float4(0.f, 0.f, 0.f, 0.f);
                }
            } else {
#pragma unroll
            for (int j = 0; j < NLD; ++j) {
                const int idx = lane + 64 * j;
                xpre[j] = make_float4(0.f, 0.f, 0.f, 0.f);
                if (ok && idx < 16 * V) {
                    const int r = idx / V, c4 = idx - r * V;
                    const unsigned row = map.tile_row((unsigned)tile, first, r, aligned);
                    xpre[j] = *reinterpret_cast<const float4 *>(ex.obs + (size_t)row * DP + 4 * c4);
                }
            }
            }
        };
        prefetch(pair_global, pl + L::kXT);
        __syncthreads();

        float *hsP = pl + L::kHT, *dsP = pl + L::kDT;
        for (int j = 0; j < J; ++j) {
            float *xs = pl + L::kXT + (j % L::kXSlots) * L::kXSlot;
            PFA_STAMP(j, 0);
            if constexpr (!kGlds) {
#pragma unroll
            for (int q = 0; q < NLD; ++q) {
                const int idx = lane + 64 * q;
                if (idx < 16 * V) {
                    const int r = idx / V, c4 = idx - r * V;
                    float2 *d = reinterpret_cast<float2 *>(xs + r * XS + 4 * c4);
                    d[0] = make_float2(xpre[q].x, xpre[q].y);
                    d[1] = make_float2(xpre[q].z, xpre[q].w);
                }
            }
            }
            const RowScalars rs = rspre;
            prefetch(pair_global + (long long)(j + 1) * pair_count, pl + L::kXT + ((j + 1) % L::kXSlots) * L::kXSlot);
            wave_lds_fence();
            PFA_STAMP(j, 1);

            f32x4 h[kMT];
            if constexpr (kPipe) {
            constexpr int NK4 = (ABL & 4) ? 0 : (KKM + 3) / 4;
            f32x4 wq[2][kMT];
            float xb[2][4];
            auto load_group = [&](int k4, int b) {
#pragma unroll
                for (int q = 0; q < 4; ++q) xb[b][q] = xs[L::xi(c, 4 * (4 * k4 + q) + g)];
#pragma unroll
                for (int m = 0; m < kMT; ++m) wq[b][m] = *reinterpret_cast<const f32x4 *>(w1t + (m * 64 + lane) * W1S + 4 * k4);
            };
            if (NK4 > 0) load_group(0, 0);
#pragma unroll
            for (int m = 0; m < kMT; ++m) h[m] = *reinterpret_cast<const f32x4 *>(b1t + (m * 64 + lane) * 4);
#pragma unroll
            for (int k4 = 0; k4 < NK4; ++k4) {
                if (k4 + 1 < NK4) load_group(k4 + 1, (k4 + 1) & 1);
                __builtin_amdgcn_sched_barrier(0);
#pragma unroll
                for (int q = 0; q < 4; ++q)
#pragma unroll
                    for (int m = 0; m < kMT; ++m)
                        if (4 * k4 + q < KKM) h[m] = mfma16(wq[k4 & 1][m][q], xb[k4 & 1][q], h[m]);
                __builtin_amdgcn_sched_barrier(0);
            }
            if constexpr (FCOL) {
                const float xcol = xs[L::xi(c, 16 * KTM)];
#pragma unroll
                for (int m = 0; m < kMT; ++m) {
                    const f32x4 wc = *reinterpret_cast<const f32x4 *>(w1t + (m * 64 + lane) * W1S + KS);
#pragma unroll
                    for (int r = 0; r < 4; ++r) h[m][r] = fmaf(wc[r], xcol, h[m][r]);
                }
            }
            } else {
#pragma unroll
            for (int m = 0; m < kMT; ++m) h[m] = *reinterpret_cast<const f32x4 *>(b1t + (m * 64 + lane) * 4);
#pragma unroll
            for (int k4 = 0; k4 < ((ABL & 4) ? 0 : (KKU + 3) / 4); ++k4) {
                float xb[4];
#pragma unroll
                for (int q = 0; q < 4; ++q) xb[q] = xs[c * XS + 4 * (4 * k4 + q) + g];
#pragma unroll
                for (int m = 0; m < kMT; ++m) {
                    const f32x4 wq = *reinterpret_cast<const f32x4 *>(w1t + (m * 64 + lane) * W1S + 4 * k4);
#pragma unroll
                    for (int q = 0; q < 4; ++q)
                        if (4 * k4 + q < KKU) h[m] = mfma16(wq[q], xb[q], h[m]);
                }
            }
            }
            f32x4 w4h[kMT];
            if constexpr (kPipe) {
#pragma unroll
                for (int m = 0; m < kMT; ++m) w4h[m] = *reinterpret_cast<const f32x4 *>(w2t + (m * 64 + lane) * 4);
                __builtin_amdgcn_sched_barrier(0);
            }
#pragma unroll
            for (int m = 0; m < kMT; ++m)
#pragma unroll
                for (int r = 0; r < 4; ++r) {
                    if constexpr (kPipe) h[m][r] = __int_as_float(max(__float_as_int(h[m][r]), 0));
                    else h[m][r] = fmaxf(h[m][r], 0.0f);
                }
            f32x4 out;
            if constexpr (kPipe) {
                f32x4 o[4] = {f32x4{bo[0], bo[1], bo[2], bo[3]}, f32x4{0.f, 0.f, 0.f, 0.f}, f32x4{0.f, 0.f, 0.f, 0.f},
                              f32x4{0.f, 0.f, 0.f, 0.f}};
#pragma unroll
                for (int m0 = 0; m0 < kMT; m0 += 4)
#pragma unroll
                    for (int r = 0; r < 4; ++r)
#pragma unroll
                        for (int q = 0; q < 4; ++q) o[q] = mfma16(w4h[m0 + q][r], h[m0 + q][r], o[q]);
                out = (o[0] + o[1]) + (o[2] + o[3]);
            } else {
                f32x4 o[4] = {f32x4{bo[0], bo[1], bo[2], bo[3]}, f32x4{0.f, 0.f, 0.f, 0.f}, f32x4{0.f, 0.f, 0.f, 0.f},
                              f32x4{0.f, 0.f, 0.f, 0.f}};
#pragma unroll
                for (int m0 = 0; m0 < kMT; m0 += 4) {
                    f32x4 w4[4];
#pragma unroll
                    for (int q = 0; q < 4; ++q) w4[q] = *reinterpret_cast<const f32x4 *>(w2t + ((m0 + q) * 64 + lane) * 4);
#pragma unroll
                    for (int r = 0; r < 4; ++r)
#pragma unroll
                        for (int q = 0; q < 4; ++q) o[q] = mfma16(w4[q][r], h[m0 + q][r], o[q]);
                }
                out = (o[0] + o[1]) + (o[2] + o[3]);
            }
            if (out[0] == 12345.678f) PFA_STAMP(j, 7);
            PFA_STAMP(j, 2);
            LossOut lo;
            if constexpr (ABL & 1) {
                lo.dout = out * rs.weight;
                lo.pg = lo.v_loss = lo.ent = lo.neg_logratio = lo.kl = lo.clipped = rs.adv;
            } else {
                lo = ppo_loss_tile<MH, !MH, PERM>(out, rs, a, heads, g, hp, adv_mean, adv_rden, inv_rows);
            }
            const f32x4 dout = lo.dout;
#pragma unroll
            for (int r = 0; r < 4; ++r) db2[r] += dout[r];
            if (g == 0) {
                stats[0] += lo.pg;
                stats[1] += lo.v_loss;
                stats[2] += lo.ent;
                stats[3] += lo.neg_logratio;
                stats[4] += lo.kl;
                stats[5] += lo.clipped;
            }
            if (stats[0] == 12345.678f) PFA_STAMP(j, 7);
            PFA_STAMP(j, 3);
            __syncthreads();
            PFA_STAMP(j, 4);
#pragma unroll
            for (int m = 0; m < kMT; ++m) *reinterpret_cast<f32x4 *>(hsP + c * HS + 16 * m + 4 * g) = h[m];
            *reinterpret_cast<f32x4 *>(dsP + c * DS + 4 * g) = dout;
            __syncthreads();
            PFA_STAMP(j, 5);
            if constexpr (kPipe) {
            if (!(ABL & 2)) {
                float dfrag[4];
                float hrow[kMT][4];
#pragma unroll
                for (int r = 0; r < 4; ++r) dfrag[r] = dsP[(4 * g + r) * DS + c];
#pragma unroll
                for (int m = 0; m < kMT; ++m)
#pragma unroll
                    for (int r = 0; r < 4; ++r) hrow[m][r] = hsP[(4 * g + r) * HS + 16 * m + c];
                __builtin_amdgcn_sched_barrier(0);
#pragma unroll
                for (int r = 0; r < 4; ++r)
#pragma unroll
                    for (int m = 0; m < kMT; ++m) acc_dw2[m] = mfma16(hrow[m][r], dfrag[r], acc_dw2[m]);
            }
            } else {
            if (!(ABL & 2)) {
                float dfrag[4];
#pragma unroll
                for (int r = 0; r < 4; ++r) dfrag[r] = dsP[(4 * g + r) * DS + c];
#pragma unroll
                for (int m0 = 0; m0 < kMT; m0 += 4) {
                    float hrow[4][4];
#pragma unroll
                    for (int q = 0; q < 4; ++q)
#pragma unroll
                        for (int r = 0; r < 4; ++r) hrow[q][r] = hsP[(4 * g + r) * HS + 16 * (m0 + q) + c];
#pragma unroll
                    for (int r = 0; r < 4; ++r)
#pragma unroll
                        for (int q = 0; q < 4; ++q) acc_dw2[m0 + q] = mfma16(hrow[q][r], dfrag[r], acc_dw2[m0 + q]);
                }
            }
            }
        }
        __syncthreads();
        __syncthreads();

#pragma unroll
        for (int r = 0; r < 4; ++r)
#pragma unroll
            for (int s = 1; s < 16; s <<= 1) db2[r] += __shfl_xor(db2[r], s, 64);
#pragma unroll
        for (int i = 0; i < 6; ++i)
#pragma unroll
            for (int s = 1; s < 16; s <<= 1) stats[i] += __shfl_xor(stats[i], s, 64);
        float *red = lds + (kQuad ? pair : (pair & 1)) * NL::kCount;
        for (int turn = 0; turn < (kQuad ? 1 : kGradPairs / 2); ++turn) {
            if (kQuad || (pair >> 1) == turn) {
                const bool first = kQuad || turn == 0;
#pragma unroll
                for (int m = 0; m < kMT; ++m)
#pragma unroll
                    for (int r = 0; r < 4; ++r) {
                        const int idx = NL::kDw2 + (m * 4 + r) * 64 + lane;
                        red[idx] = (first ? 0.0f : red[idx]) + acc_dw2[m][r];
                    }
                if (c == 0) {
#pragma unroll
                    for (int r = 0; r < 4; ++r) {
                        const int idx = NL::kDb2 + 4 * g + r;
                        red[idx] = (first ? 0.0f : red[idx]) + db2[r];
                    }
                }
                if (lane == 0) {
#pragma unroll
                    for (int i = 0; i < kNumStats; ++i) {
                        const int idx = NL::kStats + i;
                        red[idx] = (first ? 0.0f : red[idx]) + (i < 6 ? stats[i] : 0.0f);
                    }
                }
            }
            __syncthreads();
        }
    } else {
        f32x4 acc_dw1[KTM][kMT];
        float acc_col[kMT];
#pragma unroll
        for (int m = 0; m < kMT; ++m) {
#pragma unroll
            for (int kt = 0; kt < KTM; ++kt) acc_dw1[kt][m] = f32x4{0.f, 0.f, 0.f, 0.f};
            acc_col[m] = 0.0f;
        }
        __syncthreads();

        float db1[kMT];
#pragma unroll
        for (int m = 0; m < kMT; ++m) db1[m] = 0.0f;
        const float *hsP = pl + L::kHT, *dsP = pl + L::kDT;
        auto backward_tile = [&](int jj) {
            const long long tile = pair_global + (long long)jj * pair_count;
            if ((ABL & 2) || tile >= tiles) return;
            const float *xs = pl + L::kXT + (jj % L::kXSlots) * L::kXSlot;
            const f32x4 dout = *reinterpret_cast<const f32x4 *>(dsP + c * DS + 4 * g);
            float xa[KTM][4], xc[4];
#pragma unroll
            for (int r = 0; r < 4; ++r) {
#pragma unroll
                for (int kt = 0; kt < KTM; ++kt) xa[kt][r] = xs[L::xi(4 * g + r, 16 * kt + c)];
                xc[r] = COL ? xs[L::xi(4 * g + r, 16 * KTM)] : 0.0f;
            }
            if constexpr (kPipe) {
            f32x4 dh[kMT], wb[kMT];
            float hrow[kMT][4];
#pragma unroll
            for (int m = 0; m < kMT; ++m) {
                dh[m] = f32x4{0.f, 0.f, 0.f, 0.f};
                wb[m] = *reinterpret_cast<const f32x4 *>(w2bt + (m * 64 + lane) * 4);
            }
#pragma unroll
            for (int m = 0; m < kMT; ++m)
#pragma unroll
                for (int r = 0; r < 4; ++r) hrow[m][r] = hsP[(4 * g + r) * HS + 16 * m + c];
            __builtin_amdgcn_sched_barrier(0);
#pragma unroll
            for (int r = 0; r < (PERM ? 3 : 4); ++r)
#pragma unroll
                for (int m = 0; m < kMT; ++m) dh[m] = mfma16(dout[r], wb[m][r], dh[m]);
#pragma unroll
            for (int m = 0; m < kMT; ++m)
#pragma unroll
                for (int r = 0; r < 4; ++r) {
                    dh[m][r] = hrow[m][r] > 0.0f ? dh[m][r] : 0.0f;
                    db1[m] += dh[m][r];
                    if (COL) acc_col[m] = fmaf(xc[r], dh[m][r], acc_col[m]);
                }
#pragma unroll
            for (int r = 0; r < 4; ++r)
#pragma unroll
                for (int m = 0; m < kMT; ++m)
#pragma unroll
                    for (int kt = 0; kt < KTM; ++kt) acc_dw1[kt][m] = mfma16(xa[kt][r], dh[m][r], acc_dw1[kt][m]);
            } else {
#pragma unroll
            for (int m0 = 0; m0 < kMT; m0 += 4) {
                f32x4 dh[4], wb[4];
                float hrow[4][4];
#pragma unroll
                for (int q = 0; q < 4; ++q) {
                    dh[q] = f32x4{0.f, 0.f, 0.f, 0.f};
                    wb[q] = *reinterpret_cast<const f32x4 *>(w2bt + ((m0 + q) * 64 + lane) * 4);
#pragma unroll
                    for (int r = 0; r < 4; ++r) hrow[q][r] = hsP[(4 * g + r) * HS + 16 * (m0 + q) + c];
                }
#pragma unroll
                for (int r = 0; r < 4; ++r)
#pragma unroll
                    for (int q = 0; q < 4; ++q) {
                        if constexpr (DP > 64) {
                            asm volatile("v_mfma_f32_16x16x4_f32 %0, %1, %2, %0" : "+v"(dh[q]) : "v"(dout[r]), "v"(wb[q][r]));
                        } else {
                            dh[q] = mfma16(dout[r], wb[q][r], dh[q]);
                        }
                    }
                if constexpr (DP > 64) {
                    asm volatile("s_nop 7\n\ts_nop 3" ::: "memory");
                }
#pragma unroll
                for (int q = 0; q < 4; ++q)
#pragma unroll
                    for (int r = 0; r < 4; ++r) {
                        dh[q][r] = hrow[q][r] > 0.0f ? dh[q][r] : 0.0f;
                        db1[m0 + q] += dh[q][r];
                        if (COL) acc_col[m0 + q] = fmaf(xc[r], dh[q][r], acc_col[m0 + q]);
                    }
#pragma unroll
                for (int q = 0; q < 4; ++q)
#pragma unroll
                    for (int r = 0; r < 4; ++r)
#pragma unroll
                        for (int kt = 0; kt < KTM; ++kt) acc_dw1[kt][m0 + q] = mfma16(xa[kt][r], dh[q][r], acc_dw1[kt][m0 + q]);
            }
            }
        };
        for (int j = 0; j < J; ++j) {
            PFA_STAMP(j, 0);
            if (j > 0) backward_tile(j - 1);
            if (acc_dw1[0][0][0] == 12345.678f) PFA_STAMP(j, 7);
            PFA_STAMP(j, 1);
            __syncthreads();
            PFA_STAMP(j, 2);
            __syncthreads();
            PFA_STAMP(j, 3);
        }
        backward_tile(J - 1);
        __syncthreads();
        __syncthreads();

#pragma unroll
        for (int m = 0; m < kMT; ++m) {
            db1[m] += __shfl_xor(db1[m], 16, 64);
            db1[m] += __shfl_xor(db1[m], 32, 64);
            if (COL) acc_col[m] = gsum<true>(acc_col[m]);
        }
        float *red = lds + (kQuad ? pair : (pair & 1)) * NL::kCount;
        for (int turn = 0; turn < (kQuad ? 1 : kGradPairs / 2); ++turn) {
            if (kQuad || (pair >> 1) == turn) {
                const bool first = kQuad || turn == 0;
#pragma unroll
                for (int kt = 0; kt < KTM; ++kt)
#pragma unroll
                    for (int m = 0; m < kMT; ++m)
#pragma unroll
                        for (int r = 0; r < 4; ++r) {
                            const int idx = NL::kDw1 + ((kt * kMT + m) * 4 + r) * 64 + lane;
                            red[idx] = (first ? 0.0f : red[idx]) + acc_dw1[kt][m][r];
                        }
                if (g == 0) {
#pragma unroll
                    for (int m = 0; m < kMT; ++m) {
                        const int idx = NL::kDb1 + 16 * m + c;
                        red[idx] = (first ? 0.0f : red[idx]) + db1[m];
                        if (COL) {
                            const int ic = NL::kCol + 16 * m + c;
                            red[ic] = (first ? 0.0f : red[ic]) + acc_col[m];
                        }
                    }
                }
            }
            __syncthreads();
        }
    }
#ifdef PFA_DBG_SKIP_STORE
    if (blockIdx.x != 0xFFFF) return;
#endif
    float *dst = partials + (size_t)blockIdx.x * NL::kCount;
    if constexpr (kQuad) {
        for (int i = threadIdx.x; i < NL::kCount; i += kGradThreads)
            dst[i] = (lds[i] + lds[2 * NL::kCount + i]) + (lds[NL::kCount + i] + lds[3 * NL::kCount + i]);
    } else {
        for (int i = threadIdx.x; i < NL::kCount; i += kGradThreads) dst[i] = lds[i] + lds[NL::kCount + i];
    }
}

#ifndef PFA_REDUCE_SLICES
#define PFA_REDUCE_SLICES 16
#endif
constexpr int kRedSl = PFA_REDUCE_SLICES;
template <int DP, int KTM = DP / 16, bool COL = false, bool PERM = false>
__global__ void __launch_bounds__(64 * kRedSl) ppo_reduce_kernel(const float *partials, int nparts, int a, int obs_dim, float *grads,
                                                                double *norm_partials) {
    using NL = NativeLayout<DP, KTM, COL>;
    __shared__ float sh[kRedSl][64];
    __shared__ double shd[kRedSl][64];
    const int ql = threadIdx.x & 63, sl = threadIdx.x >> 6;
    const int q = blockIdx.x * 64 + ql;
    float acc = 0.0f;
    double dacc = 0.0;
    if (q < NL::kCount) {
        for (int i0 = sl; i0 < nparts; i0 += 16 * kRedSl) {
            float v[16];
#pragma unroll
            for (int u = 0; u < 16; ++u) {
                const int i = i0 + kRedSl * u;
                v[u] = i < nparts ? partials[(size_t)i * NL::kCount + q] : 0.0f;
            }
#pragma unroll
            for (int u = 0; u < 16; ++u) {
                acc += v[u];
                if (q >= NL::kStats) dacc += (double)v[u];
            }
        }
    }
    sh[sl][ql] = acc;
    shd[sl][ql] = dacc;
    __syncthreads();
    const MlpOffsets off = mlp_offsets(DP, a);
    if (sl == 1) {
        constexpr int kFirst = 16 * KTM + (COL ? 1 : 0), kPad = DP - kFirst, kDiv = kPad > 0 ? kPad : 1;
        const int e = blockIdx.x * 64 + ql;
        if (kPad > 0 && e < kHidden * kPad) grads[off.w1 + (e / kDiv) * DP + kFirst + e % kDiv] = 0.0f;
    }
    if (sl != 0) return;
    float s = 0.0f;
    int p = -1;
    if (q < NL::kCount) {
        float t[kRedSl];
#pragma unroll
        for (int w = 0; w < kRedSl; ++w) t[w] = sh[w][ql];
#pragma unroll
        for (int w = kRedSl / 2; w > 0; w >>= 1)
#pragma unroll
            for (int x = 0; x < w; ++x) t[x] += t[x + w];
        s = t[0];
        if (COL && q >= NL::kCol && q < NL::kDw2) {
            p = off.w1 + (q - NL::kCol) * DP + 16 * KTM;
            if (16 * KTM >= obs_dim) s = 0.0f;
        } else if (q < NL::kCol) {
            const int ln = q & 63, r = (q >> 6) & 3, m = (q >> 8) & (kMT - 1), kt = q >> 11;
            p = off.w1 + (16 * m + (ln & 15)) * DP + 16 * kt + 4 * (ln >> 4) + r;
            if (16 * kt + 4 * (ln >> 4) + r >= obs_dim) s = 0.0f;
        } else if (q < NL::kDb1) {
            const int t = q - NL::kDw2, ln = t & 63, r = (t >> 6) & 3, m = t >> 8;
            const int o = slot_output(PERM, ln & 15), u = 16 * m + 4 * (ln >> 4) + r;
            if (o < a) p = off.w2 + o * kHidden + u;
            else if (o == a) p = off.wv + u;
        } else if (q < NL::kDb2) {
            p = off.b1 + (q - NL::kDb1);
        } else if (q < NL::kStats) {
            const int o = slot_output(PERM, q - NL::kDb2);
            if (o < a) p = off.b2 + o;
            else if (o == a) p = off.bv;
        } else {
            double t = 0.0;
#pragma unroll
            for (int w = 0; w < kRedSl; ++w) t += shd[w][ql];
            const float hi = (float)t;
            grads[off.count + 2 * (q - NL::kStats)] = hi;
            grads[off.count + 2 * (q - NL::kStats) + 1] = (float)(t - (double)hi);
        }
        if (p >= 0) grads[p] = s;
    }
    double sq = (p >= 0 && p < off.count) ? (double)s * (double)s : 0.0;
#pragma unroll
    for (int o = 32; o > 0; o >>= 1) sq += __shfl_xor(sq, o, 64);
    if (ql == 0) norm_partials[blockIdx.x] = sq;
}

__device__ __forceinline__ void adam_element(float &p, float &m, float &v, float g, float clip, float neg_step_size, float bc2_sqrt,
                                             float beta1, float beta2, float eps) {
#pragma clang fp contract(off)
    const float w1 = 1.0f - beta1, w2 = 1.0f - beta2;
    const float gi = g * clip;
    m = m + w1 * (gi - m);
    v = (v * beta2) + ((w2 * gi) * gi);
    const float denom = (sqrtf(v) / bc2_sqrt) + eps;
    p = p + ((neg_step_size * m) / denom);
}
__device__ __forceinline__ float clip_factor(double sum_sq, float max_grad_norm) {
#pragma clang fp contract(off)
    const float total_norm = (float)sqrt(sum_sq);
    if (!(max_grad_norm > 0.0f)) return 1.0f;
    const float clip = max_grad_norm / (total_norm + 1e-6f);
    return clip > 1.0f ? 1.0f : clip;
}

constexpr int kAdamThreads = 256;

struct GridWords {
    unsigned long long *words;
    unsigned gen;
    int *status;
    long long timeout_ticks;
};
struct AdamArgs {
    float *params, *exp_avg, *exp_avg_sq;
    float neg_step_size, bc2_sqrt, beta1, beta2, eps, max_grad_norm;
    double *losses;
    double loss_scale;
    const double *log_ev4;
    double *log_out10;
};
template <int DP, int KTM, bool COL, bool PERM, bool DIST>
__global__ void __launch_bounds__(64 * kRedSl) ppo_reduce_adam_kernel(const float *partials, int nparts, int a, int obs_dim, float *grads,
                                                                     GridWords gw, AdamArgs ad, LlArgs ll) {
    using NL = NativeLayout<DP, KTM, COL>;
    __shared__ float sh[kRedSl][64];
    __shared__ double shd[kRedSl][64];
    const int ql = threadIdx.x & 63, sl = threadIdx.x >> 6;
    const int q = blockIdx.x * 64 + ql;
    const bool status_lane = DIST && blockIdx.x == 0 && threadIdx.x == 0;
    int status_mine = 0;
    if constexpr (DIST) {
        if (status_lane) status_mine = ll_status_push(ll);
    }
    float acc = 0.0f;
    double dacc = 0.0;
    if (q < NL::kCount) {
        for (int i0 = sl; i0 < nparts; i0 += 16 * kRedSl) {
            float v[16];
#pragma unroll
            for (int u = 0; u < 16; ++u) {
                const int i = i0 + kRedSl * u;
                v[u] = i < nparts ? partials[(size_t)i * NL::kCount + q] : 0.0f;
            }
#pragma unroll
            for (int u = 0; u < 16; ++u) {
                acc += v[u];
                if (q >= NL::kStats) dacc += (double)v[u];
            }
        }
    }
    sh[sl][ql] = acc;
    shd[sl][ql] = dacc;
    __syncthreads();
    const MlpOffsets off = mlp_offsets(DP, a);
    if (sl == 1) {
        constexpr int kFirst = 16 * KTM + (COL ? 1 : 0), kPad = DP - kFirst, kDiv = kPad > 0 ? kPad : 1;
        const int e = blockIdx.x * 64 + ql;
        if (kPad > 0 && e < kHidden * kPad) grads[off.w1 + (e / kDiv) * DP + kFirst + e % kDiv] = 0.0f;
    }
    if (sl != 0) return;
    float s = 0.0f, hi = 0.0f, lo = 0.0f;
    int p = -1;
    const bool stat = q >= NL::kStats && q < NL::kCount;
    if (q < NL::kCount) {
        float t[kRedSl];
#pragma unroll
        for (int w = 0; w < kRedSl; ++w) t[w] = sh[w][ql];
#pragma unroll
        for (int w = kRedSl / 2; w > 0; w >>= 1)
#pragma unroll
            for (int x = 0; x < w; ++x) t[x] += t[x + w];
        s = t[0];
        if (COL && q >= NL::kCol && q < NL::kDw2) {
            p = off.w1 + (q - NL::kCol) * DP + 16 * KTM;
            if (16 * KTM >= obs_dim) s = 0.0f;
        } else if (q < NL::kCol) {
            const int ln = q & 63, r = (q >> 6) & 3, m = (q >> 8) & (kMT - 1), kt = q >> 11;
            p = off.w1 + (16 * m + (ln & 15)) * DP + 16 * kt + 4 * (ln >> 4) + r;
            if (16 * kt + 4 * (ln >> 4) + r >= obs_dim) s = 0.0f;
        } else if (q < NL::kDb1) {
            const int t2 = q - NL::kDw2, ln = t2 & 63, r = (t2 >> 6) & 3, m = t2 >> 8;
            const int o = slot_output(PERM, ln & 15), u = 16 * m + 4 * (ln >> 4) + r;
            if (o < a) p = off.w2 + o * kHidden + u;
            else if (o == a) p = off.wv + u;
        } else if (q < NL::kDb2) {
            p = off.b1 + (q - NL::kDb1);
        } else if (q < NL::kStats) {
            const int o = slot_output(PERM, q - NL::kDb2);
            if (o < a) p = off.b2 + o;
            else if (o == a) p = off.bv;
        } else {
            double t2 = 0.0;
#pragma unroll
            for (int w = 0; w < kRedSl; ++w) t2 += shd[w][ql];
            hi = (float)t2;
            lo = (float)(t2 - (double)hi);
        }
    }
    float p_i = 0.0f, m_i = 0.0f, v_i = 0.0f;
    if (p >= 0) {
        p_i = ad.params[p];
        m_i = ad.exp_avg[p];
        v_i = ad.exp_avg_sq[p];
    }
    if constexpr (DIST) {
        if (p >= 0) ll_push(ll, (unsigned)q, s);
        if (stat) {
            ll_push(ll, (unsigned)(NL::kStats + 2 * (q - NL::kStats)), hi);
            ll_push(ll, (unsigned)(NL::kStats + 2 * (q - NL::kStats) + 1), lo);
        }
        long long waited = 0;
        if (p >= 0) s = ll_wait_sum(ll, (unsigned)q, s, &waited);
        if (stat) {
            hi = ll_wait_sum(ll, (unsigned)(NL::kStats + 2 * (q - NL::kStats)), hi, &waited);
            lo = ll_wait_sum(ll, (unsigned)(NL::kStats + 2 * (q - NL::kStats) + 1), lo, &waited);
        }
        ll_wait_report(ll, waited);
    }
    if (p >= 0) grads[p] = s;
    if (stat) {
        grads[off.count + 2 * (q - NL::kStats)] = hi;
        grads[off.count + 2 * (q - NL::kStats) + 1] = lo;
    }
    double sq = (p >= 0 && p < off.count) ? (double)s * (double)s : 0.0;
#pragma unroll
    for (int o = 32; o > 0; o >>= 1) sq += __shfl_xor(sq, o, 64);
    if (ql < 2) {
        const unsigned long long bits = (unsigned long long)__double_as_longlong(sq);
        const unsigned half = ql == 0 ? (unsigned)bits : (unsigned)(bits >> 32);
        __hip_atomic_store(gw.words + 2 * blockIdx.x + ql, ((unsigned long long)gw.gen << 32) | half, __ATOMIC_RELAXED, __HIP_MEMORY_SCOPE_AGENT);
    }
    if constexpr (DIST) {
        if (status_lane) ll_status_wait(ll, status_mine);
    }
    const int npart = (int)gridDim.x;
    double tot = 0.0;
#pragma unroll
    for (int w = 0; w < kAdamThreads / 64; ++w) {
        double ss = 0.0;
        for (int i = 64 * w + ql; i < npart; i += kAdamThreads) {
            unsigned long long w0, w1;
            long long t0 = 0;
            int spin = 0;
            bool lost = false;
            while (true) {
                w0 = __hip_atomic_load(gw.words + 2 * i, __ATOMIC_RELAXED, __HIP_MEMORY_SCOPE_AGENT);
                w1 = __hip_atomic_load(gw.words + 2 * i + 1, __ATOMIC_RELAXED, __HIP_MEMORY_SCOPE_AGENT);
                if ((unsigned)(w0 >> 32) == gw.gen && (unsigned)(w1 >> 32) == gw.gen) break;
                __builtin_amdgcn_s_sleep(1);
                if ((++spin & 255) == 0) {
                    const long long now = (long long)wall_clock64();
                    if (t0 == 0) t0 = now;
                    else if (now - t0 > gw.timeout_ticks) {
                        lost = true;
                        break;
                    }
                }
            }
            if (lost) {
                __hip_atomic_store(gw.status, 1, __ATOMIC_RELAXED, __HIP_MEMORY_SCOPE_SYSTEM);
                ss = __builtin_nan("");
                break;
            }
            ss += __longlong_as_double((long long)(((w1 & 0xffffffffull) << 32) | (w0 & 0xffffffffull)));
        }
#pragma unroll
        for (int o = 32; o > 0; o >>= 1) ss += __shfl_xor(ss, o, 64);
        tot += ss;
    }
    const float clip = clip_factor(tot, ad.max_grad_norm);
    if (p >= 0) {
        adam_element(p_i, m_i, v_i, s, clip, ad.neg_step_size, ad.bc2_sqrt, ad.beta1, ad.beta2, ad.eps);
        ad.params[p] = p_i;
        ad.exp_avg[p] = m_i;
        ad.exp_avg_sq[p] = v_i;
    }
    if (stat) {
        const int i = q - NL::kStats;
        double run = 0.0;
        if (ad.losses && i < 6) {
            run = ad.losses[i] + ((double)hi + (double)lo) * ad.loss_scale;
            ad.losses[i] = run;
        }
        if (ad.log_out10) {
            static_assert(kNumStats == 8, "slots 6 and 7 carry the four explained-variance sums of the report");
            if (i < 6) {
                ad.log_out10[i] = run;
            } else {
                ad.log_out10[6 + 2 * (i - 6)] = ad.log_ev4[2 * (i - 6)];
                ad.log_out10[7 + 2 * (i - 6)] = ad.log_ev4[2 * (i - 6) + 1];
            }
        }
    }
}

constexpr int kAdvChunks = 64;
__global__ void __launch_bounds__(256) adv_stats_partial_kernel(const float *adv, RowMap base, long long mb_rows,
                                                               double *partial ) {
    __shared__ double sh1[256], sh2[256];
    RowMap map = base;
    map.mb = blockIdx.y;
    const long long per = (mb_rows + kAdvChunks - 1) / kAdvChunks;
    const long long lo = (long long)blockIdx.x * per, hi = lo + per < mb_rows ? lo + per : mb_rows;
    double s1 = 0.0, s2 = 0.0;
    for (long long q = lo + threadIdx.x; q < hi; q += 256) {
        const double v = (double)adv[map.flat(q)];
        s1 += v;
        s2 += v * v;
    }
    sh1[threadIdx.x] = s1;
    sh2[threadIdx.x] = s2;
    __syncthreads();
    for (int s = 128; s > 0; s >>= 1) {
        if ((int)threadIdx.x < s) {
            sh1[threadIdx.x] += sh1[threadIdx.x + s];
            sh2[threadIdx.x] += sh2[threadIdx.x + s];
        }
        __syncthreads();
    }
    if (threadIdx.x == 0) {
        partial[((size_t)blockIdx.y * kAdvChunks + blockIdx.x) * 2 + 0] = sh1[0];
        partial[((size_t)blockIdx.y * kAdvChunks + blockIdx.x) * 2 + 1] = sh2[0];
    }
}
__global__ void adv_stats_final_kernel(const double *partial, int nmb, double *stats) {
    const int mb = blockIdx.x * blockDim.x + threadIdx.x;
    if (mb >= nmb) return;
    double s1 = 0.0, s2 = 0.0;
    for (int i = 0; i < kAdvChunks; ++i) {
        s1 += partial[((size_t)mb * kAdvChunks + i) * 2 + 0];
        s2 += partial[((size_t)mb * kAdvChunks + i) * 2 + 1];
    }
    stats[2 * mb] = s1;
    stats[2 * mb + 1] = s2;
}

constexpr int kEvBlocks = 128;
__global__ void __launch_bounds__(256) ev_partial_kernel(const float *adv, const float *values, long long n, int num_envs,
                                                        int horizon, double *partial ) {
    __shared__ double sh[4][256];
    double a[4] = {0, 0, 0, 0};
    for (long long j = (long long)blockIdx.x * 256 + threadIdx.x; j < n; j += (long long)kEvBlocks * 256) {
        const long long e = j % num_envs, t = j / num_envs;
        const double yp = (double)values[e * horizon + t];
        const double ad = (double)adv[j];
        const double yt = ad + yp;
        a[0] += yt;
        a[1] += yt * yt;
        a[2] += ad;
        a[3] += ad * ad;
    }
    for (int q = 0; q < 4; ++q) sh[q][threadIdx.x] = a[q];
    __syncthreads();
    for (int s = 128; s > 0; s >>= 1) {
        if ((int)threadIdx.x < s)
            for (int q = 0; q < 4; ++q) sh[q][threadIdx.x] += sh[q][threadIdx.x + s];
        __syncthreads();
    }
    if (threadIdx.x < 4) partial[blockIdx.x * 4 + threadIdx.x] = sh[threadIdx.x][0];
}
__global__ void ev_final_kernel(const double *partial, const double *losses, double *out10) {
    const int q = threadIdx.x;
    if (q < 6) out10[q] = losses ? losses[q] : 0.0;
    if (q >= 6 && q < 10) {
        double s = 0.0;
        for (int b = 0; b < kEvBlocks; ++b) s += partial[b * 4 + (q - 6)];
        out10[q] = s;
    }
}

__global__ void __launch_bounds__(kAdamThreads) adam_clip_kernel(float *params, const float *grads, float *exp_avg,
                                                                float *exp_avg_sq, long long count, float neg_step_size,
                                                                float bc2_sqrt, float beta1, float beta2, float eps,
                                                                float max_grad_norm, float grad_scale, const float *loss_sums,
                                                                double *losses, double loss_scale, const double *norm_partials,
                                                                int n_norm_partials) {
    __shared__ double sh[kAdamThreads / 64];
    const long long i = (long long)blockIdx.x * kAdamThreads + threadIdx.x;
    float g_i = 0.0f, m = 0.0f, v = 0.0f, p_i = 0.0f;
    if (i < count) {
        g_i = grads[i];
        m = exp_avg[i];
        v = exp_avg_sq[i];
        p_i = params[i];
    }
    double ss = 0.0;
    if (norm_partials) {
        for (int i = threadIdx.x; i < n_norm_partials; i += kAdamThreads) ss += norm_partials[i];
        ss *= (double)grad_scale * (double)grad_scale;
    } else {
        for (long long base = threadIdx.x; base < count; base += kAdamThreads * 8) {
            float gv[8];
#pragma unroll
            for (int u = 0; u < 8; ++u) {
                const long long i = base + (long long)u * kAdamThreads;
                gv[u] = i < count ? grads[i] * grad_scale : 0.0f;
            }
#pragma unroll
            for (int u = 0; u < 8; ++u) ss += (double)gv[u] * (double)gv[u];
        }
    }
#pragma unroll
    for (int off = 32; off > 0; off >>= 1) ss += __shfl_xor(ss, off, 64);
    if (lane_id() == 0) sh[wave_id()] = ss;
    __syncthreads();
    double tot = 0.0;
#pragma unroll
    for (int w = 0; w < kAdamThreads / 64; ++w) tot += sh[w];
    const float clip = clip_factor(tot, max_grad_norm);
    if (i < count) {
        adam_element(p_i, m, v, g_i * grad_scale, clip, neg_step_size, bc2_sqrt, beta1, beta2, eps);
        params[i] = p_i;
        exp_avg[i] = m;
        exp_avg_sq[i] = v;
    }
    if (blockIdx.x == 0 && loss_sums && losses && threadIdx.x < 6)
        losses[threadIdx.x] += ((double)loss_sums[2 * threadIdx.x] + (double)loss_sums[2 * threadIdx.x + 1]) * loss_scale;
}

static int check_update_args(const pfa_experience *ex, int64_t batch_rows, const pfa_mlp_dims *dims,
                             const pfa_ppo_hparams *hp) {
    PFA_REQUIRE(ex && hp, "ppo: null argument");
    PFA_REQUIRE(hp->num_minibatches >= 1 && hp->bptt_horizon >= 1, "ppo: bad minibatch partition");
    PFA_REQUIRE(batch_rows % hp->num_minibatches == 0, "batch_size must be divisible by minibatch_size");
    const int64_t mbs = batch_rows / hp->num_minibatches;
    PFA_REQUIRE(mbs % hp->bptt_horizon == 0, "minibatch_size must be divisible by bptt_horizon");
    (void)dims;
    return 0;
}

static bool grad_trimmed(const pfa_mlp_dims *dims) { return dims->obs_stride == 64 && !dims->heads && dims->obs_dim == 49; }
#ifndef PFA_GRAD_PERM
#define PFA_GRAD_PERM 1
#endif
static bool grad_perm(const pfa_mlp_dims *dims) { return PFA_GRAD_PERM && dims->num_actions <= 11; }
static bool grad_bf16(const pfa_mlp_dims *dims, int64_t mbs) { return pfa_igemm_get_products() == 1 && grad_trimmed(dims) && mbs >= 32 && mbs % 32 == 0; }
static int norm_blocks(const pfa_mlp_dims *dims) {
    const int count = grad_trimmed(dims) ? NativeLayout<64, 3, true>::kCount
                                         : (dims->obs_stride / 16) * kMT * 4 * 64 + kMT * 4 * 64 + kHidden + kOut + kNumStats;
    return (count + 63) / 64;
}
static size_t native_count(int dp) { return (size_t)(dp / 16) * kMT * 4 * 64 + kMT * 4 * 64 + kHidden + kOut + kNumStats; }
static size_t partials_bytes(const pfa_mlp_dims *dims) {
    return align_up((size_t)(dims->obs_stride == 64 ? kBfMaxGrid : 256) * native_count(dims->obs_stride) * sizeof(float), 256);
}
static double *norm_partials_of(void *workspace, const pfa_mlp_dims *dims) {
    return (double *)((char *)workspace + partials_bytes(dims));
}
constexpr size_t kGridWordsBytes = 16384;
static size_t tail_bytes(const pfa_mlp_dims *dims, int nmb) {
    const size_t native = native_count(dims->obs_stride);
    const size_t advp = align_up((size_t)nmb * 64 * 2 * sizeof(double), 256);
    const size_t normp = align_up(((native + 63) / 64) * 2 * sizeof(double), 256);
    return advp > normp ? advp : normp;
}


static int grad_grid(int64_t mb_rows, int dp) {
    const int64_t tiles = mb_rows / 16;
    const int64_t wgs = (tiles + grad_pairs(dp) - 1) / grad_pairs(dp);
    return (int)(wgs < 256 ? (wgs < 1 ? 1 : wgs) : 256);
}

}

using namespace pfa;

extern "C" size_t pfa_ppo_workspace_bytes(const pfa_mlp_dims *dims, int64_t batch_rows, const pfa_ppo_hparams *hp) {
    if (!dims || !hp || hp->num_minibatches < 1) return 0;
    (void)batch_rows;
    static_assert(kAdvChunks == 64, "tail_bytes assumes 64 chunks");
    return partials_bytes(dims) + tail_bytes(dims, hp->num_minibatches) + 256;
}

extern "C" int pfa_ppo_adv_stats(const pfa_experience *exp, int64_t batch_rows, const pfa_ppo_hparams *hp, double *stats,
                                 void *workspace, pfa_stream_t stream) {
    if (int rc = check_update_args(exp, batch_rows, nullptr, hp)) return rc;
    PFA_REQUIRE(exp->advantages && stats && workspace, "ppo.adv_stats: null buffer");
    const int64_t mbs = batch_rows / hp->num_minibatches;
    RowMap map{0, hp->num_minibatches, hp->bptt_horizon};
    double *partial = (double *)workspace;
    hipLaunchKernelGGL(adv_stats_partial_kernel, dim3(kAdvChunks, hp->num_minibatches), dim3(256), 0, (hipStream_t)stream,
                       exp->advantages, map, (long long)mbs, partial);
    PFA_LAUNCH_CHECK();
    hipLaunchKernelGGL(adv_stats_final_kernel, dim3((hp->num_minibatches + 63) / 64), dim3(64), 0, (hipStream_t)stream, partial,
                       hp->num_minibatches, stats);
    PFA_LAUNCH_CHECK();
    return 0;
}

static int launch_grad(const pfa_experience *exp, int64_t batch_rows, int32_t mb, const float *params,
                       const pfa_mlp_dims *dims, const pfa_ppo_hparams *hp, const double *adv_stats,
                       int64_t global_mb_rows, float *grads, void *workspace, pfa_stream_t stream, int *grid_out) {
    if (int rc = check_update_args(exp, batch_rows, dims, hp)) return rc;
    PFA_REQUIRE(dims && dims->hidden == kHidden, "ppo.grad: hidden must be %d", kHidden);
    PFA_REQUIRE(dims->obs_stride == 16 || dims->obs_stride == 32 || dims->obs_stride == 64 || dims->obs_stride == 96 ||
                    dims->obs_stride == 128,
                "ppo.grad: obs_stride must be 16/32/64/96/128");
    PFA_REQUIRE(dims->num_actions >= 1 && dims->num_actions <= 15, "ppo.grad: num_actions must be in 1..15");
    PFA_REQUIRE(dims->heads == 0 || heads_count(dims->heads, dims->num_actions) >= 1, "ppo.grad: head sizes 0x%x do not sum to num_actions %d",
                dims->heads, dims->num_actions);
    PFA_REQUIRE(mb >= 0 && mb < hp->num_minibatches, "ppo.grad: minibatch index out of range");
    PFA_REQUIRE(exp->obs && exp->actions && exp->logprobs && exp->values && exp->advantages && exp->returns && params && grads &&
                    workspace,
                "ppo.grad: null buffer");
    PFA_REQUIRE(!hp->norm_adv || adv_stats, "ppo.grad: norm_adv needs adv_stats");
    const int64_t mbs = batch_rows / hp->num_minibatches;
    PFA_REQUIRE(mbs % 16 == 0, "ppo.grad: minibatch_size must be a multiple of 16 (got %lld)", (long long)mbs);
    PFA_REQUIRE(global_mb_rows >= mbs, "ppo.grad: global_mb_rows < local minibatch rows");
    RowMap map{mb, hp->num_minibatches, hp->bptt_horizon};
    float *partials = (float *)workspace;
    if (grad_bf16(dims, mbs)) {
        const int64_t tiles32 = mbs / 32;
        const int grid = (int)(tiles32 < kBfMaxGrid ? tiles32 : kBfMaxGrid);
        hipEvent_t ev0 = nullptr, ev1 = nullptr;
        const bool timed = timing_pair("ppo_mlp_grad", &ev0, &ev1);
        ScopedKernelTimer timer(timing_ext_mode() ? nullptr : "ppo_mlp_grad", (hipStream_t)stream);
#define PFA_LAUNCH_GRAD_BF16(PERMV)                                                                                                       \
    {                                                                                                                                    \
        static bool attr_set = false;                                                                                                    \
        if (!attr_set) {                                                                                                                 \
            PFA_CHECK_HIP(hipFuncSetAttribute((const void *)ppo_mlp_grad_bf16_kernel<PERMV>, hipFuncAttributeMaxDynamicSharedMemorySize,  \
                                              (int)BfLds::kBytes));                                                                      \
            attr_set = true;                                                                                                             \
        }                                                                                                                                \
        if (timed)                                                                                                                       \
            hipExtLaunchKernelGGL((ppo_mlp_grad_bf16_kernel<PERMV>), dim3(grid), dim3(kBfThreads), BfLds::kBytes, (hipStream_t)stream,    \
                                  ev0, ev1, 0, *exp, map, (long long)mbs, params, dims->num_actions, *hp, adv_stats,                     \
                                  (double)global_mb_rows, partials);                                                                     \
        else                                                                                                                             \
            hipLaunchKernelGGL((ppo_mlp_grad_bf16_kernel<PERMV>), dim3(grid), dim3(kBfThreads), BfLds::kBytes, (hipStream_t)stream, *exp, \
                               map, (long long)mbs, params, dims->num_actions, *hp, adv_stats, (double)global_mb_rows, partials);        \
    }
        if (grad_perm(dims)) PFA_LAUNCH_GRAD_BF16(true)
        else PFA_LAUNCH_GRAD_BF16(false)
#undef PFA_LAUNCH_GRAD_BF16
        PFA_LAUNCH_CHECK();
        *grid_out = grid;
        return 0;
    }
    const int grid = grad_grid(mbs, dims->obs_stride);
#define PFA_LAUNCH_GRAD_FULL(DPV, KKUV, MHV, KTMV, COLV) PFA_LAUNCH_GRAD_PERM(DPV, KKUV, MHV, KTMV, COLV, false)
#define PFA_LAUNCH_GRAD_PERM(DPV, KKUV, MHV, KTMV, COLV, PERMV)                                                             \
    {                                                                                                                      \
        constexpr size_t lds_bytes = (size_t)GradLds<DPV, grad_glds(DPV, KTMV)>::kFloats * sizeof(float);                       \
        static_assert((size_t)2 * NativeLayout<DPV, KTMV, COLV>::kCount * sizeof(float) <= lds_bytes,                       \
                      "the two reduction buffers must fit in the tile/table area");                                       \
        static bool attr_set = false;                                                                                      \
        if (!attr_set) {                                                                                                   \
            PFA_CHECK_HIP(hipFuncSetAttribute((const void *)ppo_mlp_grad_kernel<DPV, 0, KKUV, MHV, KTMV, COLV, PERMV>,     \
                                              hipFuncAttributeMaxDynamicSharedMemorySize, (int)lds_bytes));                \
            attr_set = true;                                                                                               \
        }                                                                                                                  \
        if (grad_timed)                                                                                                    \
            hipExtLaunchKernelGGL((ppo_mlp_grad_kernel<DPV, 0, KKUV, MHV, KTMV, COLV, PERMV>), dim3(grid), dim3(grad_threads(DPV)), \
                                  lds_bytes, (hipStream_t)stream, grad_ev0, grad_ev1, 0, *exp, map, (long long)mbs, params,  \
                                  dims->num_actions, dims->heads, *hp, adv_stats, (double)global_mb_rows, partials);      \
        else                                                                                                               \
            hipLaunchKernelGGL((ppo_mlp_grad_kernel<DPV, 0, KKUV, MHV, KTMV, COLV, PERMV>), dim3(grid), dim3(grad_threads(DPV)), \
                               lds_bytes, (hipStream_t)stream, *exp, map, (long long)mbs, params, dims->num_actions,       \
                               dims->heads, *hp, adv_stats, (double)global_mb_rows, partials);                             \
    }
#define PFA_LAUNCH_GRAD_KM(DPV, KKUV, MHV) PFA_LAUNCH_GRAD_FULL(DPV, KKUV, MHV, DPV / 16, false)
#define PFA_LAUNCH_GRAD_K(DPV, KKUV) PFA_LAUNCH_GRAD_KM(DPV, KKUV, false)
#define PFA_LAUNCH_GRAD(DPV)                                        \
    if (dims->heads) PFA_LAUNCH_GRAD_KM(DPV, DPV / 4, true)         \
    else PFA_LAUNCH_GRAD_KM(DPV, DPV / 4, false)
    {
        hipEvent_t grad_ev0 = nullptr, grad_ev1 = nullptr;
        const bool grad_timed = timing_pair("ppo_mlp_grad", &grad_ev0, &grad_ev1);
        ScopedKernelTimer timer(timing_ext_mode() ? nullptr : "ppo_mlp_grad", (hipStream_t)stream);
        switch (dims->obs_stride) {
            case 16: PFA_LAUNCH_GRAD(16) break;
            case 32: PFA_LAUNCH_GRAD(32) break;
            case 96: PFA_LAUNCH_GRAD(96) break;
            case 128: PFA_LAUNCH_GRAD(128) break;
            default:
                if (grad_trimmed(dims) && grad_perm(dims)) PFA_LAUNCH_GRAD_PERM(64, 13, false, 3, true, true)
                else if (grad_trimmed(dims)) PFA_LAUNCH_GRAD_FULL(64, 13, false, 3, true)
                else if (!dims->heads && (dims->obs_dim + 3) / 4 == 13) PFA_LAUNCH_GRAD_K(64, 13)
                else PFA_LAUNCH_GRAD(64)
                break;
        }
    }
#undef PFA_LAUNCH_GRAD_KM
#undef PFA_LAUNCH_GRAD_FULL
#undef PFA_LAUNCH_GRAD_PERM
#undef PFA_LAUNCH_GRAD
#undef PFA_LAUNCH_GRAD_K
    PFA_LAUNCH_CHECK();
    *grid_out = grid;
    return 0;
}

extern "C" int pfa_ppo_mlp_grad(const pfa_experience *exp, int64_t batch_rows, int32_t mb, const float *params,
                                const pfa_mlp_dims *dims, const pfa_ppo_hparams *hp, const double *adv_stats,
                                int64_t global_mb_rows, float *grads, void *workspace, pfa_stream_t stream) {
    int grid = 0;
    if (int rc = launch_grad(exp, batch_rows, mb, params, dims, hp, adv_stats, global_mb_rows, grads, workspace, stream, &grid)) return rc;
    float *partials = (float *)workspace;
    double *normp = norm_partials_of(workspace, dims);
    ScopedKernelTimer timer2("ppo_reduce", (hipStream_t)stream);
#define PFA_LAUNCH_REDUCE(DPV, KTMV, COLV) PFA_LAUNCH_REDUCE_P(DPV, KTMV, COLV, false)
#define PFA_LAUNCH_REDUCE_P(DPV, KTMV, COLV, PERMV)                                                                             \
    hipLaunchKernelGGL((ppo_reduce_kernel<DPV, KTMV, COLV, PERMV>), dim3((NativeLayout<DPV, KTMV, COLV>::kCount + 63) / 64),     \
                       dim3(64 * kRedSl), 0, (hipStream_t)stream, partials, grid, dims->num_actions, dims->obs_dim, grads, normp)
    switch (dims->obs_stride) {
        case 16: PFA_LAUNCH_REDUCE(16, 1, false); break;
        case 32: PFA_LAUNCH_REDUCE(32, 2, false); break;
        case 96: PFA_LAUNCH_REDUCE(96, 6, false); break;
        case 128: PFA_LAUNCH_REDUCE(128, 8, false); break;
        default:
            if (grad_trimmed(dims) && grad_perm(dims)) PFA_LAUNCH_REDUCE_P(64, 3, true, true);
            else if (grad_trimmed(dims)) PFA_LAUNCH_REDUCE(64, 3, true);
            else PFA_LAUNCH_REDUCE(64, 4, false);
            break;
    }
#undef PFA_LAUNCH_REDUCE
#undef PFA_LAUNCH_REDUCE_P
    PFA_LAUNCH_CHECK();
    return 0;
}

extern "C" int pfa_ppo_mlp_grad_path(const pfa_mlp_dims *dims, int64_t mb_rows) { return dims && grad_bf16(dims, mb_rows) ? 1 : 0; }

extern "C" int pfa_ppo_mlp_grad_mfma_per_tile(int32_t obs_dim, int32_t obs_stride, int32_t num_actions) {
    if (num_actions < 1 || num_actions > 15) return 0;
    if (obs_stride != 16 && obs_stride != 32 && obs_stride != 64 && obs_stride != 96 && obs_stride != 128) return 0;
    int kku = obs_stride / 4, ktm = obs_stride / 16;
    if (obs_stride == 64 && (obs_dim + 3) / 4 == 13) kku = 13;
    if (obs_stride == 64 && obs_dim == 49) ktm = 3;
    if (PFA_GRAD_FCOL && obs_stride == 64 && obs_dim == 49) kku = 12;
    const bool perm = PFA_GRAD_PERM && obs_stride == 64 && obs_dim == 49 && num_actions <= 11;
    return kku * kMT + (perm ? 11 : 12) * kMT + ktm * 4 * kMT;
}

extern "C" int pfa_adam_clip_step(float *params, const float *grads, float *exp_avg, float *exp_avg_sq, int64_t count, float lr,
                                  float beta1, float beta2, float eps, int64_t step, float max_grad_norm, float grad_scale,
                                  const float *loss_sums, double *losses, double loss_scale, const double *norm_partials,
                                  int32_t n_norm_partials, pfa_stream_t stream) {
    PFA_REQUIRE(params && grads && exp_avg && exp_avg_sq, "adam: null buffer");
    PFA_REQUIRE(count >= 1 && step >= 1, "adam: count and step must be >= 1");
    const double bc1 = 1.0 - std::pow((double)beta1, (double)step);
    const double bc2 = 1.0 - std::pow((double)beta2, (double)step);
    const float neg_step_size = (float)(-(double)lr / bc1);
    const float bc2_sqrt = (float)std::sqrt(bc2);
    ScopedKernelTimer timer("adam_clip", (hipStream_t)stream);
    hipLaunchKernelGGL(adam_clip_kernel, dim3((unsigned)((count + kAdamThreads - 1) / kAdamThreads)), dim3(kAdamThreads), 0,
                       (hipStream_t)stream, params, grads, exp_avg, exp_avg_sq, (long long)count, neg_step_size, bc2_sqrt, beta1,
                       beta2, eps, max_grad_norm, grad_scale, loss_sums, losses, loss_scale, norm_partials, (int)n_norm_partials);
    PFA_LAUNCH_CHECK();
    return 0;
}

static unsigned long long *grid_words_of(void *workspace) {
    static std::unordered_map<void *, unsigned long long *> words;
    auto it = words.find(workspace);
    if (it != words.end()) return it->second;
    if (words.size() >= 64) {
        (void)hipDeviceSynchronize();
        for (auto &kv : words) (void)hipFree(kv.second);
        words.clear();
    }
    void *p = nullptr;
    if (hipMalloc(&p, kGridWordsBytes) != hipSuccess) return nullptr;
    if (hipMemset(p, 0, kGridWordsBytes) != hipSuccess || hipDeviceSynchronize() != hipSuccess) {
        (void)hipFree(p);
        return nullptr;
    }
    words[workspace] = (unsigned long long *)p;
    return (unsigned long long *)p;
}
static int *grid_status_word() {
    static int *word = nullptr;
    if (!word) {
        void *p = nullptr;
        if (hipHostMalloc(&p, 64, hipHostMallocMapped) != hipSuccess) return nullptr;
        *(volatile int *)p = 0;
        word = (int *)p;
    }
    return word;
}
static long long grid_timeout_ticks() {
    static const long long ticks = [] {
        long long ms = 10000;
        if (const char *e = std::getenv("PFA_WAIT_TIMEOUT_MS")) {
            const long long v = std::atoll(e);
            if (v > 0) ms = v;
        }
        return ms * 100000;
    }();
    return ticks;
}
template <typename K>
static bool coresident(K kernel, int blocks) {
    int per_cu = 0, cus = 0, dev = 0;
    if (hipGetDevice(&dev) != hipSuccess) return false;
    if (hipDeviceGetAttribute(&cus, hipDeviceAttributeMultiprocessorCount, dev) != hipSuccess) return false;
    if (hipOccupancyMaxActiveBlocksPerMultiprocessor(&per_cu, (const void *)kernel, 64 * kRedSl, 0) != hipSuccess) return false;
    return (long long)per_cu * cus >= blocks;
}
static bool reduce_adam_coresident(const pfa_mlp_dims *dims, bool dist) {
    static int cache[2][8] = {};
    const int slot = dims->obs_stride == 16 ? 0 : dims->obs_stride == 32 ? 1 : dims->obs_stride == 96 ? 2 : dims->obs_stride == 128 ? 3
                   : (grad_trimmed(dims) && grad_perm(dims)) ? 4 : grad_trimmed(dims) ? 5 : 6;
    int &c = cache[dist ? 1 : 0][slot];
    if (c) return c == 1;
    const int blocks = norm_blocks(dims);
    bool ok;
#define PFA_CO(DPV, KTMV, COLV, PERMV) \
    ok = dist ? coresident(ppo_reduce_adam_kernel<DPV, KTMV, COLV, PERMV, true>, blocks) : coresident(ppo_reduce_adam_kernel<DPV, KTMV, COLV, PERMV, false>, blocks)
    switch (slot) {
        case 0: PFA_CO(16, 1, false, false); break;
        case 1: PFA_CO(32, 2, false, false); break;
        case 2: PFA_CO(96, 6, false, false); break;
        case 3: PFA_CO(128, 8, false, false); break;
        case 4: PFA_CO(64, 3, true, true); break;
        case 5: PFA_CO(64, 3, true, false); break;
        default: PFA_CO(64, 4, false, false); break;
    }
#undef PFA_CO
    c = ok ? 1 : 2;
    return ok;
}
static int launch_reduce_adam(const pfa_mlp_dims *dims, int nmb, int grid, float *params, float *grads, float *exp_avg, float *exp_avg_sq,
                              float lr, float beta1, float beta2, float eps, int64_t step, float max_grad_norm, double *losses,
                              double loss_scale, void *workspace, const LlArgs *ll, hipStream_t stream, const double *log_ev4 = nullptr,
                              double *log_out10 = nullptr) {
    const double bc1 = 1.0 - std::pow((double)beta1, (double)step);
    const double bc2 = 1.0 - std::pow((double)beta2, (double)step);
    AdamArgs ad{params, exp_avg, exp_avg_sq, (float)(-(double)lr / bc1), (float)std::sqrt(bc2), beta1, beta2, eps, max_grad_norm, losses, loss_scale,
                log_ev4, log_out10};
    const float *partials = (const float *)workspace;
    static unsigned long long launches = 0;
    unsigned gen = (unsigned)(++launches);
    if (gen == 0) gen = (unsigned)(++launches);
    int *gstatus = grid_status_word();
    PFA_REQUIRE(gstatus, "ppo.train: cannot allocate the grid hand-off's status word");
    unsigned long long *gwords = grid_words_of(workspace);
    PFA_REQUIRE(gwords, "ppo.train: cannot allocate the grid hand-off words");
    PFA_REQUIRE((size_t)((native_count(dims->obs_stride) + 63) / 64) * 2 * sizeof(unsigned long long) <= kGridWordsBytes, "ppo.train: hand-off words too small");
    (void)nmb;
    const GridWords gw{gwords, gen, gstatus, grid_timeout_ticks()};
    const LlArgs none{};
    ScopedKernelTimer timer("ppo_reduce_adam", stream);
#define PFA_LAUNCH_RA(DPV, KTMV, COLV, PERMV)                                                                                        \
    {                                                                                                                               \
        const dim3 g((NativeLayout<DPV, KTMV, COLV>::kCount + 63) / 64), b(64 * kRedSl);                                            \
        if (ll) hipLaunchKernelGGL((ppo_reduce_adam_kernel<DPV, KTMV, COLV, PERMV, true>), g, b, 0, stream, partials, grid,          \
                                   dims->num_actions, dims->obs_dim, grads, gw, ad, *ll);                                   \
        else hipLaunchKernelGGL((ppo_reduce_adam_kernel<DPV, KTMV, COLV, PERMV, false>), g, b, 0, stream, partials, grid,            \
                                dims->num_actions, dims->obs_dim, grads, gw, ad, none);                                     \
    }
    switch (dims->obs_stride) {
        case 16: PFA_LAUNCH_RA(16, 1, false, false) break;
        case 32: PFA_LAUNCH_RA(32, 2, false, false) break;
        case 96: PFA_LAUNCH_RA(96, 6, false, false) break;
        case 128: PFA_LAUNCH_RA(128, 8, false, false) break;
        default:
            if (grad_trimmed(dims) && grad_perm(dims)) PFA_LAUNCH_RA(64, 3, true, true)
            else if (grad_trimmed(dims)) PFA_LAUNCH_RA(64, 3, true, false)
            else PFA_LAUNCH_RA(64, 4, false, false)
            break;
    }
#undef PFA_LAUNCH_RA
    PFA_LAUNCH_CHECK();
    return 0;
}
static size_t ll_entries_needed(const pfa_mlp_dims *dims) { return native_count(dims->obs_stride) + kTailFloats + 1; }
static bool env_on(const char *name, bool dflt) {
    const char *e = std::getenv(name);
    return e ? e[0] != '0' : dflt;
}

extern "C" int pfa_ppo_grid_status(void) {
    int *w = grid_status_word();
    return w ? *(volatile int *)w : 0;
}
extern "C" int pfa_ppo_grid_reset(void) {
    int *w = grid_status_word();
    if (!w) return 0;
    const int was = *(volatile int *)w;
    *(volatile int *)w = 0;
    return was;
}

extern "C" int pfa_ppo_mlp_train_logged(const pfa_experience *exp, int64_t batch_rows, float *params, const pfa_mlp_dims *dims,
                                        const pfa_ppo_hparams *hp, const double *adv_stats, float *grads, float *exp_avg,
                                        float *exp_avg_sq, int64_t opt_step, float lr, float beta1, float beta2, float eps,
                                        float max_grad_norm, int32_t update_epochs, double *losses, void *workspace,
                                        int32_t data_parallel, const double *log_ev4, double *log_out10, int32_t *log_packed,
                                        pfa_stream_t stream);
extern "C" int pfa_ppo_mlp_train(const pfa_experience *exp, int64_t batch_rows, float *params, const pfa_mlp_dims *dims,
                                 const pfa_ppo_hparams *hp, const double *adv_stats, float *grads, float *exp_avg,
                                 float *exp_avg_sq, int64_t opt_step, float lr, float beta1, float beta2, float eps,
                                 float max_grad_norm, int32_t update_epochs, double *losses, void *workspace,
                                 int32_t data_parallel, pfa_stream_t stream) {
    return pfa_ppo_mlp_train_logged(exp, batch_rows, params, dims, hp, adv_stats, grads, exp_avg, exp_avg_sq, opt_step, lr, beta1, beta2, eps,
                                    max_grad_norm, update_epochs, losses, workspace, data_parallel, nullptr, nullptr, nullptr, stream);
}

extern "C" int pfa_ppo_mlp_train_logged(const pfa_experience *exp, int64_t batch_rows, float *params, const pfa_mlp_dims *dims,
                                        const pfa_ppo_hparams *hp, const double *adv_stats, float *grads, float *exp_avg,
                                        float *exp_avg_sq, int64_t opt_step, float lr, float beta1, float beta2, float eps,
                                        float max_grad_norm, int32_t update_epochs, double *losses, void *workspace,
                                        int32_t data_parallel, const double *log_ev4, double *log_out10, int32_t *log_packed,
                                        pfa_stream_t stream) {
    if (log_packed) *log_packed = 0;
    PFA_REQUIRE(!log_out10 || (log_ev4 && losses), "ppo.train: the report needs the explained-variance sums and the loss accumulator");
    if (int rc = check_update_args(exp, batch_rows, dims, hp)) return rc;
    PFA_REQUIRE(update_epochs >= 0 && opt_step >= 0, "ppo.train: bad epoch / step count");
    PFA_REQUIRE(!data_parallel || dist_ready(), "ppo.train: data_parallel needs pfa_dist_init first");
    const int world = data_parallel ? dist_world() : 1;
    const int64_t mbs = batch_rows / hp->num_minibatches;
    const int64_t global_mbs = mbs * world;
    const int64_t count = mlp_offsets(dims->obs_stride, dims->num_actions).count;
    const double loss_scale = 1.0 / ((double)global_mbs * hp->num_minibatches);
    const bool fused_dp_wanted = data_parallel && world > 1 && env_on("PFA_FUSED_DP", true) && p2p_ll_ready(ll_entries_needed(dims));
    const bool fused = env_on("PFA_FUSED_ADAM", true) && reduce_adam_coresident(dims, fused_dp_wanted);
    const bool fused_dp = fused && fused_dp_wanted;
    const bool one_launch = fused && (!data_parallel || fused_dp);
    for (int e = 0; e < update_epochs; ++e)
        for (int mb = 0; mb < hp->num_minibatches; ++mb) {
            if (one_launch) {
                int grid = 0;
                if (int rc = launch_grad(exp, batch_rows, mb, params, dims, hp, adv_stats, global_mbs, grads, workspace, stream, &grid)) return rc;
                ++opt_step;
                LlArgs ll{};
                if (fused_dp) ll = p2p_ll_next();
                const bool last = log_out10 && e == update_epochs - 1 && mb == hp->num_minibatches - 1;
                if (int rc = launch_reduce_adam(dims, hp->num_minibatches, grid, params, grads, exp_avg, exp_avg_sq, lr, beta1, beta2, eps,
                                                opt_step, max_grad_norm, losses, loss_scale, workspace, fused_dp ? &ll : nullptr,
                                                (hipStream_t)stream, last ? log_ev4 : nullptr, last ? log_out10 : nullptr))
                    return rc;
                if (last && log_packed) *log_packed = 1;
                continue;
            }
            if (int rc = pfa_ppo_mlp_grad(exp, batch_rows, mb, params, dims, hp, adv_stats, global_mbs, grads, workspace, stream))
                return rc;
            ++opt_step;
            if (data_parallel) {
                if (int rc = dist_all_reduce(grads, (size_t)count + kTailFloats, false, (hipStream_t)stream)) return rc;
                if (int rc = pfa_adam_clip_step(params, grads, exp_avg, exp_avg_sq, count, lr, beta1, beta2, eps, opt_step,
                                                max_grad_norm, 1.0f, grads + count, losses, loss_scale, nullptr, 0, stream))
                    return rc;
            } else if (int rc = pfa_adam_clip_step(params, grads, exp_avg, exp_avg_sq, count, lr, beta1, beta2, eps, opt_step,
                                                   max_grad_norm, 1.0f, grads + count, losses, loss_scale,
                                                   norm_partials_of(workspace, dims),
                                                   norm_blocks(dims), stream)) {
                return rc;
            }
        }
    return 0;
}

#ifdef PFA_BF16_TRACE
extern "C" int pfa_probe_bf16_trace(unsigned long long *buf, int tiles) {
    PFA_CHECK_HIP(hipMemcpyToSymbol(HIP_SYMBOL(g_bf_trace), &buf, sizeof(buf)));
    PFA_CHECK_HIP(hipMemcpyToSymbol(HIP_SYMBOL(g_bf_trace_tiles), &tiles, sizeof(tiles)));
    return 0;
}
#endif
#ifdef PFA_PROBES
extern "C" int pfa_probe_set_trace(unsigned long long *buf, int tiles) {
    PFA_CHECK_HIP(hipMemcpyToSymbol(HIP_SYMBOL(g_trace), &buf, sizeof(buf)));
    PFA_CHECK_HIP(hipMemcpyToSymbol(HIP_SYMBOL(g_trace_tiles), &tiles, sizeof(tiles)));
    return 0;
}
extern "C" int pfa_probe_grad(const pfa_experience *exp, int64_t batch_rows, int32_t mb, const float *params,
                              const pfa_mlp_dims *dims, const pfa_ppo_hparams *hp, const double *adv_stats, float *grads,
                              void *workspace, int32_t abl, pfa_stream_t stream) {
    const int64_t mbs = batch_rows / hp->num_minibatches;
    const int grid = grad_grid(mbs, 64);
    RowMap map{mb, hp->num_minibatches, hp->bptt_horizon};
    float *partials = (float *)workspace;
    constexpr size_t lds_bytes = (size_t)GradLds<64, grad_glds(64, 3)>::kFloats * sizeof(float);
#define PFA_PROBE_CASE(A)                                                                                              \
    case A:                                                                                                            \
        PFA_CHECK_HIP(hipFuncSetAttribute((const void *)ppo_mlp_grad_kernel<64, A, 13, false, 3, true>,                                \
                                          hipFuncAttributeMaxDynamicSharedMemorySize, (int)lds_bytes));                \
        hipLaunchKernelGGL((ppo_mlp_grad_kernel<64, A, 13, false, 3, true>), dim3(grid), dim3(grad_threads(64)), lds_bytes, (hipStream_t)stream, \
                           *exp, map, (long long)mbs, params, dims->num_actions, 0u, *hp, adv_stats, (double)mbs, partials); \
        break;
    switch (abl) {
        PFA_PROBE_CASE(0) PFA_PROBE_CASE(1) PFA_PROBE_CASE(2) PFA_PROBE_CASE(4) PFA_PROBE_CASE(6) PFA_PROBE_CASE(7)
        default: return -2;
    }
#undef PFA_PROBE_CASE
    PFA_LAUNCH_CHECK();
    (void)grads;
    return 0;
}
#endif

extern "C" int pfa_train_log_sums(const pfa_experience *exp, int64_t batch_rows, int32_t num_envs, const double *losses,
                                  double *out10, void *workspace, pfa_stream_t stream) {
    PFA_REQUIRE(exp && exp->advantages && exp->values && out10 && workspace, "train_log_sums: null buffer");
    PFA_REQUIRE(num_envs >= 1 && batch_rows % num_envs == 0, "train_log_sums: batch must be whole rollout steps");
    double *partial = (double *)workspace;
    hipLaunchKernelGGL(ev_partial_kernel, dim3(kEvBlocks), dim3(256), 0, (hipStream_t)stream, exp->advantages, exp->values,
                       (long long)batch_rows, (int)num_envs, (int)(batch_rows / num_envs), partial);
    PFA_LAUNCH_CHECK();
    hipLaunchKernelGGL(ev_final_kernel, dim3(1), dim3(64), 0, (hipStream_t)stream, partial, losses, out10);
    PFA_LAUNCH_CHECK();
    return 0;
}

__global__ void ev_final4_kernel(const double *partial, double *out4) {
    const int q = threadIdx.x;
    if (q < 4) {
        double s = 0.0;
        for (int b = 0; b < kEvBlocks; ++b) s += partial[b * 4 + q];
        out4[q] = s;
    }
}
__global__ void log_pack_kernel(const double *losses, const double *ev4, double *out10) {
    const int q = threadIdx.x;
    if (q < 6) out10[q] = losses ? losses[q] : 0.0;
    else if (q < 10) out10[q] = ev4[q - 6];
}
extern "C" int pfa_train_ev_sums(const pfa_experience *exp, int64_t batch_rows, int32_t num_envs, double *out4, void *workspace,
                                 pfa_stream_t stream) {
    PFA_REQUIRE(exp && exp->advantages && exp->values && out4 && workspace, "train_ev_sums: null buffer");
    PFA_REQUIRE(num_envs >= 1 && batch_rows % num_envs == 0, "train_ev_sums: batch must be whole rollout steps");
    double *partial = (double *)workspace;
    hipLaunchKernelGGL(ev_partial_kernel, dim3(kEvBlocks), dim3(256), 0, (hipStream_t)stream, exp->advantages, exp->values,
                       (long long)batch_rows, (int)num_envs, (int)(batch_rows / num_envs), partial);
    PFA_LAUNCH_CHECK();
    hipLaunchKernelGGL(ev_final4_kernel, dim3(1), dim3(64), 0, (hipStream_t)stream, partial, out4);
    PFA_LAUNCH_CHECK();
    return 0;
}
extern "C" int pfa_train_log_pack(const double *losses, const double *ev4, double *out10, pfa_stream_t stream) {
    PFA_REQUIRE(ev4 && out10, "train_log_pack: null buffer");
    hipLaunchKernelGGL(log_pack_kernel, dim3(1), dim3(64), 0, (hipStream_t)stream, losses, ev4, out10);
    PFA_LAUNCH_CHECK();
    return 0;
}
```

Baseline: 418.1 million env_steps/s.

## Add sparse-observation gather path for the PPO MLP gradient first layer

Adds a scan kernel that runs once per update and encodes each observation row as at most two nonzero (index, value) pairs. It raises a device flag if any row is denser than that or holds a non-finite value. A new GATHER variant of the gradient kernel then computes the first hidden layer by reading two W1 rows from an LDS-transposed table instead of doing the dense obs×W1 product, and stages x late only for the backward pass. Both the dense and the gather kernels are launched every minibatch and each exits early according to the device flag, so correctness never depends on the data. The cost is an extra scan pass, extra workspace, and one empty kernel launch per minibatch.

Measured after the change: 459.8 million env_steps/s (median of 6 runs). +10.0%, better.

```diff
diff --git a/include/pufferlib_amd.h b/include/pufferlib_amd.h
--- a/include/pufferlib_amd.h
+++ b/include/pufferlib_amd.h
@@ -234,6 +234,8 @@
 } pfa_ppo_hparams;
 
 size_t pfa_ppo_workspace_bytes(const pfa_mlp_dims *dims, int64_t batch_rows, const pfa_ppo_hparams *hp);
+int pfa_ppo_obs_scan_result(const void *workspace, const pfa_mlp_dims *dims, const pfa_ppo_hparams *hp, int64_t batch_rows,
+                            int32_t *dense_needed);
 int pfa_ppo_adv_stats(const pfa_experience *exp, int64_t batch_rows, const pfa_ppo_hparams *hp,
                       double *stats, void *workspace, pfa_stream_t stream);
 int pfa_ppo_mlp_grad(const pfa_experience *exp, int64_t batch_rows, int32_t mb, const float *params,
diff --git a/pufferlib_amd/_lib.py b/pufferlib_amd/_lib.py
--- a/pufferlib_amd/_lib.py
+++ b/pufferlib_amd/_lib.py
@@ -205,6 +205,7 @@
     'pfa_multiagent_episode_stats': (C.c_int, [P, C.c_int32, P, C.c_int32, P]),
     'pfa_nativize_rows': (C.c_int, [P, C.c_int64, C.c_int32, P, C.c_int32, P]),
     'pfa_ppo_workspace_bytes': (C.c_size_t, [C.POINTER(MlpDims), C.c_int64, C.POINTER(PpoHparams)]),
+    'pfa_ppo_obs_scan_result': (C.c_int, [P, C.POINTER(MlpDims), C.POINTER(PpoHparams), C.c_int64, C.POINTER(C.c_int32)]),
     'pfa_ppo_adv_stats': (C.c_int, [C.POINTER(Experience), C.c_int64, C.POINTER(PpoHparams), P, P, P]),
     'pfa_ppo_mlp_grad': (C.c_int, [C.POINTER(Experience), C.c_int64, C.c_int32, P, C.POINTER(MlpDims),
                                    C.POINTER(PpoHparams), P, C.c_int64, P, P, P]),
diff --git a/pufferlib_amd/csrc/ppo_tile.hpp b/pufferlib_amd/csrc/ppo_tile.hpp
--- a/pufferlib_amd/csrc/ppo_tile.hpp
+++ b/pufferlib_amd/csrc/ppo_tile.hpp
@@ -84,6 +84,11 @@
 struct RowScalars {
     int action;
     float old_logprob, old_value, adv, ret, weight;
+};
+
+struct __attribute__((aligned(16))) ObsCode {
+    float v0, v1;
+    int k0, k1;
 };
 
 struct LossOut {
diff --git a/pufferlib_amd/csrc/ppo_update.hip b/pufferlib_amd/csrc/ppo_update.hip
--- a/pufferlib_amd/csrc/ppo_update.hip
+++ b/pufferlib_amd/csrc/ppo_update.hip
@@ -85,10 +85,14 @@
 __host__ __device__ constexpr int slot_output(bool perm, int slot) {
     return !perm ? slot : ((slot & 3) == 3 ? 99 : 3 * (slot >> 2) + (slot & 3));
 }
-template <int DP, int ABL = 0, int KKU = DP / 4, bool MH = false, int KTM = DP / 16, bool COL = false, bool PERM = false>
-__global__ void __launch_bounds__(grad_threads(DP), grad_waves_per_simd(DP))
-    ppo_mlp_grad_kernel(pfa_experience ex, RowMap map, long long mb_rows, const float *params, int a, uint32_t heads,
-                        pfa_ppo_hparams hp, const double *adv_stats , double global_rows, float *partials) {
+constexpr int kGatherStride = kHidden + 4;
+constexpr bool grad_can_gather(int dp, int abl, int kku, bool mh, int ktm, bool col) {
+    return dp == 64 && abl == 0 && kku == 13 && !mh && ktm == 3 && col;
+}
+template <int DP, int ABL, int KKU, bool MH, int KTM, bool COL, bool PERM, bool GATHER>
+__device__ __forceinline__ void ppo_mlp_grad_body(const pfa_experience &ex, const RowMap &map, long long mb_rows, const float *params, int a,
+                                                  uint32_t heads, const pfa_ppo_hparams &hp, const double *adv_stats ,
+                                                  double global_rows, float *partials, const ObsCode *codes) {
     constexpr bool kGlds = grad_glds(DP, KTM);
     using L = GradLds<DP, kGlds>;
     using NL = NativeLayout<DP, KTM, COL>;
@@ -126,6 +130,22 @@
             tw[j] = w2v_at(params, off, a, slot_output(PERM, cc), 16 * m + 4 * gg + r);
             tv[j] = w2v_at(params, off, a, slot_output(PERM, 4 * gg + r), 16 * m + cc);
         }
+        if constexpr (GATHER) {
+            static_assert(DP * kGatherStride <= L::kW1Floats && (DP & (DP - 1)) == 0, "the W1^T table sits in the fragment table's area");
+            constexpr int NG = kHidden * DP / kGradThreads;
+            static_assert(kHidden * DP % kGradThreads == 0, "table sizes");
+            float tg[NG];
+#pragma unroll
+            for (int j = 0; j < NG; ++j) {
+                const int i = threadIdx.x + j * kGradThreads;
+                tg[j] = params[off.w1 + i];
+            }
+#pragma unroll
+            for (int j = 0; j < NG; ++j) {
+                const int i = threadIdx.x + j * kGradThreads;
+                w1t[(i % DP) * kGatherStride + i / DP] = tg[j];
+            }
+        } else {
 #pragma unroll 1
         for (int j0 = 0; j0 < N1; j0 += CH) {
             float t1[CH];
@@ -141,6 +161,7 @@
                 const int kk = i % KS, ln = (i / KS) & 63, m = i / (KS * 64);
                 w1t[(m * 64 + ln) * W1S + kk] = t1[j];
             }
+        }
         }
 #pragma unroll
         for (int j = 0; j < N2; ++j) {
@@ -149,7 +170,7 @@
             w2t[i] = tw[j];
             w2bt[i] = tv[j];
         }
-        if constexpr (FCOL) {
+        if constexpr (FCOL && !GATHER) {
             static_assert(W1S - KS >= 4 && KS % 4 == 0, "the trailing-column fragment sits in the lane's pad floats");
             float tc[N2];
 #pragma unroll
@@ -167,6 +188,10 @@
     }
 #endif
 
+    auto fresh_lane = [&]() -> int {
+        if constexpr (GATHER) return (int)__builtin_amdgcn_mbcnt_hi(~0u, __builtin_amdgcn_mbcnt_lo(~0u, 0u));
+        else return lane;
+    };
     const long long tiles = mb_rows / 16;
     const long long pair_global = (long long)blockIdx.x * kGradPairs + pair;
     const long long pair_count = (long long)gridDim.x * kGradPairs;
@@ -200,13 +225,18 @@
 
         float4 xpre[kGlds ? 1 : NLD];
         RowScalars rspre;
-        auto prefetch = [&](long long tile, float *xdst) {
+        ObsCode cdpre;
+        auto prefetch = [&](long long tile, float *xdst, bool scalars = true, bool xrows = true) {
             const bool ok = tile < tiles;
             const unsigned first = ok ? map.tile_first((unsigned)tile) : 0u;
+            if (scalars) {
             rspre = RowScalars{0, 0.f, 0.f, 0.f, 0.f, 0.f};
-            if (ok) {
+            if constexpr (GATHER) cdpre = ObsCode{0.f, 0.f, 0, 1};
+            }
+            if (scalars && ok) {
                 const unsigned fr = map.tile_row((unsigned)tile, first, c, aligned);
                 rspre = RowScalars{ex.actions[fr], ex.logprobs[fr], ex.values[fr], ex.advantages[fr], ex.returns[fr], 1.0f};
+                if constexpr (GATHER) cdpre = codes[fr];
             }
             if constexpr (kGlds) {
                 const int kl = lane >> 4, row = (lane & 12) + ((lane - kl) & 3);
@@ -220,7 +250,7 @@
 #pragma unroll
                     for (int b = 0; b < DP / 16; ++b) *reinterpret_cast<float4 *>(xdst + 256 * b + 4 * lane) = make_float4(0.f, 0.f, 0.f, 0.f);
                 }
-            } else {
+            } else if (xrows) {
 #pragma unroll
             for (int j = 0; j < NLD; ++j) {
                 const int idx = lane + 64 * j;
@@ -240,7 +270,8 @@
         for (int j = 0; j < J; ++j) {
             float *xs = pl + L::kXT + (j % L::kXSlots) * L::kXSlot;
             PFA_STAMP(j, 0);
-            if constexpr (!kGlds) {
+            constexpr bool kLateX = GATHER && !kGlds;
+            auto stage_x = [&]() {
 #pragma unroll
             for (int q = 0; q < NLD; ++q) {
                 const int idx = lane + 64 * q;
@@ -251,14 +282,36 @@
                     d[1] = make_float2(xpre[q].z, xpre[q].w);
                 }
             }
-            }
+            };
+            if constexpr (!kGlds && !kLateX) stage_x();
             const RowScalars rs = rspre;
-            prefetch(pair_global + (long long)(j + 1) * pair_count, pl + L::kXT + ((j + 1) % L::kXSlots) * L::kXSlot);
+            ObsCode cd;
+            if constexpr (GATHER) cd = cdpre;
+            prefetch(pair_global + (long long)(j + 1) * pair_count, pl + L::kXT + ((j + 1) % L::kXSlots) * L::kXSlot, true, !kLateX);
             wave_lds_fence();
             PFA_STAMP(j, 1);
 
             f32x4 h[kMT];
-            if constexpr (kPipe) {
+            if constexpr (GATHER) {
+            const float *w0 = w1t + (cd.k0 & (DP - 1)) * kGatherStride + 4 * g, *w1 = w1t + (cd.k1 & (DP - 1)) * kGatherStride + 4 * g;
+            f32x4 wa[kMT];
+#pragma unroll
+            for (int m = 0; m < kMT; ++m) {
+                h[m] = *reinterpret_cast<const f32x4 *>(b1t + (m * 64 + lane) * 4);
+                wa[m] = *reinterpret_cast<const f32x4 *>(w0 + 16 * m);
+            }
+#pragma unroll
+            for (int m = 0; m < kMT; ++m)
+#pragma unroll
+                for (int r = 0; r < 4; ++r) h[m][r] = fmaf(wa[m][r], cd.v0, h[m][r]);
+            __builtin_amdgcn_sched_barrier(0);
+#pragma unroll
+            for (int m = 0; m < kMT; ++m) wa[m] = *reinterpret_cast<const f32x4 *>(w1 + 16 * m);
+#pragma unroll
+            for (int m = 0; m < kMT; ++m)
+#pragma unroll
+                for (int r = 0; r < 4; ++r) h[m][r] = fmaf(wa[m][r], cd.v1, h[m][r]);
+            } else if constexpr (kPipe) {
             constexpr int NK4 = (ABL & 4) ? 0 : (KKM + 3) / 4;
             f32x4 wq[2][kMT];
             float xb[2][4];
@@ -349,6 +402,7 @@
             }
             if (out[0] == 12345.678f) PFA_STAMP(j, 7);
             PFA_STAMP(j, 2);
+            if constexpr (kLateX) stage_x();
             LossOut lo;
             if constexpr (ABL & 1) {
                 lo.dout = out * rs.weight;
@@ -376,6 +430,7 @@
             *reinterpret_cast<f32x4 *>(dsP + c * DS + 4 * g) = dout;
             __syncthreads();
             PFA_STAMP(j, 5);
+            if constexpr (kLateX) prefetch(pair_global + (long long)(j + 1) * pair_count, nullptr, false, true);
             if constexpr (kPipe) {
             if (!(ABL & 2)) {
                 float dfrag[4];
@@ -603,12 +658,30 @@
     if (blockIdx.x != 0xFFFF) return;
 #endif
     float *dst = partials + (size_t)blockIdx.x * NL::kCount;
+    const int tid = GATHER ? wv * 64 + fresh_lane() : (int)threadIdx.x;
     if constexpr (kQuad) {
-        for (int i = threadIdx.x; i < NL::kCount; i += kGradThreads)
+        for (int i = tid; i < NL::kCount; i += kGradThreads)
             dst[i] = (lds[i] + lds[2 * NL::kCount + i]) + (lds[NL::kCount + i] + lds[3 * NL::kCount + i]);
     } else {
-        for (int i = threadIdx.x; i < NL::kCount; i += kGradThreads) dst[i] = lds[i] + lds[NL::kCount + i];
-    }
+        for (int i = tid; i < NL::kCount; i += kGradThreads) dst[i] = lds[i] + lds[NL::kCount + i];
+    }
+}
+
+constexpr int kSparseHeaderInts = 64;
+constexpr int kSparseMinEpochs = 2;
+template <int DP, int ABL = 0, int KKU = DP / 4, bool MH = false, int KTM = DP / 16, bool COL = false, bool PERM = false, bool GATHER = false>
+__global__ void __launch_bounds__(grad_threads(DP), grad_waves_per_simd(DP))
+    ppo_mlp_grad_kernel(pfa_experience ex, RowMap map, long long mb_rows, const float *params, int a, uint32_t heads,
+                        pfa_ppo_hparams hp, const double *adv_stats , double global_rows, float *partials,
+                        const int *sparse) {
+    static_assert(!GATHER || grad_can_gather(DP, ABL, KKU, MH, KTM, COL), "the gather form exists for the trimmed 64-float instantiations");
+    if constexpr (GATHER) {
+        if (!sparse || *sparse != 0) return;
+    } else if constexpr (grad_can_gather(DP, ABL, KKU, MH, KTM, COL)) {
+        if (sparse && *sparse == 0) return;
+    }
+    ppo_mlp_grad_body<DP, ABL, KKU, MH, KTM, COL, PERM, GATHER>(ex, map, mb_rows, params, a, heads, hp, adv_stats, global_rows, partials,
+                                                                GATHER ? reinterpret_cast<const ObsCode *>(sparse + kSparseHeaderInts) : nullptr);
 }
 
 #ifndef PFA_REDUCE_SLICES
@@ -1028,6 +1101,54 @@
         losses[threadIdx.x] += ((double)loss_sums[2 * threadIdx.x] + (double)loss_sums[2 * threadIdx.x + 1]) * loss_scale;
 }
 
+constexpr int kScanRows = 4, kScanThreads = 256, kScanBlockRows = kScanThreads / 16 * kScanRows;
+__global__ void __launch_bounds__(kScanThreads) obs_sparse_scan_kernel(const float *obs, long long rows, int obs_dim, ObsCode *codes,
+                                                                       int *dense_needed) {
+    const int l = threadIdx.x & 15, grp = threadIdx.x >> 4, lane = threadIdx.x & 63;
+    const long long row0 = (long long)blockIdx.x * kScanBlockRows + grp * kScanRows;
+    float4 x[kScanRows];
+#pragma unroll
+    for (int i = 0; i < kScanRows; ++i) {
+        x[i] = make_float4(0.f, 0.f, 0.f, 0.f);
+        if (row0 + i < rows) x[i] = *reinterpret_cast<const float4 *>(obs + (size_t)(row0 + i) * 64 + 4 * l);
+    }
+    bool bad = false;
+#pragma unroll
+    for (int i = 0; i < kScanRows; ++i) {
+        const float xs[4] = {x[i].x, x[i].y, x[i].z, x[i].w};
+        int n = 0, ka = 0, kb = 0;
+        float va = 0.f, vb = 0.f;
+#pragma unroll
+        for (int q = 0; q < 4; ++q) {
+            const int k = 4 * l + q;
+            if (k < obs_dim && xs[q] != 0.0f) {
+                if (n == 0) { ka = k; va = xs[q]; }
+                if (n == 1) { kb = k; vb = xs[q]; }
+                ++n;
+                bad |= !(fabsf(xs[q]) <= 3.402823466e38f);
+            }
+        }
+        const unsigned long long ball = __ballot(n > 0), b2 = __ballot(n > 1), b3 = __ballot(n > 2);
+        const int sh = lane & 48;
+        const unsigned has = (unsigned)(ball >> sh) & 0xFFFFu, two = (unsigned)(b2 >> sh) & 0xFFFFu, three = (unsigned)(b3 >> sh) & 0xFFFFu;
+        const int total = __popc(has) + __popc(two) + (three ? 2 : 0);
+        const int la = has ? __ffs(has) - 1 : 0;
+        const unsigned rest = has & (has - 1);
+        const int lb = rest ? __ffs(rest) - 1 : la;
+        const int src = sh + la, src2 = sh + lb;
+        const int k0 = __shfl(ka, src, 64), kb0 = __shfl(kb, src, 64), k1o = __shfl(ka, src2, 64);
+        const float v0 = __shfl(va, src, 64), vb0 = __shfl(vb, src, 64), v1o = __shfl(va, src2, 64);
+        bad |= total > 2;
+        if (l == 0 && row0 + i < rows) {
+            ObsCode cd{0.f, 0.f, 0, 1};
+            if (total == 1) cd = k0 == 0 ? ObsCode{v0, 0.f, 0, 1} : ObsCode{0.f, v0, 0, k0};
+            else if (total == 2) cd = (two & (1u << la)) ? ObsCode{v0, vb0, k0, kb0} : ObsCode{v0, v1o, k0, k1o};
+            codes[row0 + i] = cd;
+        }
+    }
+    if (bad) *dense_needed = 1;
+}
+
 static int check_update_args(const pfa_experience *ex, int64_t batch_rows, const pfa_mlp_dims *dims,
                              const pfa_ppo_hparams *hp) {
     PFA_REQUIRE(ex && hp, "ppo: null argument");
@@ -1064,7 +1185,10 @@
     const size_t normp = align_up(((native + 63) / 64) * 2 * sizeof(double), 256);
     return advp > normp ? advp : normp;
 }
-
+static size_t sparse_offset(const pfa_mlp_dims *dims, int nmb) { return partials_bytes(dims) + tail_bytes(dims, nmb) + 256; }
+static size_t sparse_bytes(const pfa_mlp_dims *dims, int64_t batch_rows) {
+    return grad_trimmed(dims) && batch_rows > 0 ? kSparseHeaderInts * sizeof(int) + (size_t)batch_rows * sizeof(ObsCode) : 0;
+}
 
 static int grad_grid(int64_t mb_rows, int dp) {
     const int64_t tiles = mb_rows / 16;
@@ -1078,9 +1202,20 @@
 
 extern "C" size_t pfa_ppo_workspace_bytes(const pfa_mlp_dims *dims, int64_t batch_rows, const pfa_ppo_hparams *hp) {
     if (!dims || !hp || hp->num_minibatches < 1) return 0;
-    (void)batch_rows;
     static_assert(kAdvChunks == 64, "tail_bytes assumes 64 chunks");
-    return partials_bytes(dims) + tail_bytes(dims, hp->num_minibatches) + 256;
+    return sparse_offset(dims, hp->num_minibatches) + sparse_bytes(dims, batch_rows);
+}
+
+extern "C" int pfa_ppo_obs_scan_result(const void *workspace, const pfa_mlp_dims *dims, const pfa_ppo_hparams *hp, int64_t batch_rows,
+                                       int32_t *dense_needed) {
+    PFA_REQUIRE(workspace && dims && hp && dense_needed && hp->num_minibatches >= 1, "ppo.obs_scan_result: null argument");
+    *dense_needed = 1;
+    if (!sparse_bytes(dims, batch_rows)) return 0;
+    int word = 1;
+    PFA_CHECK_HIP(hipDeviceSynchronize());
+    PFA_CHECK_HIP(hipMemcpy(&word, (const char *)workspace + sparse_offset(dims, hp->num_minibatches), sizeof(word), hipMemcpyDeviceToHost));
+    *dense_needed = word != 0;
+    return 0;
 }
 
 extern "C" int pfa_ppo_adv_stats(const pfa_experience *exp, int64_t batch_rows, const pfa_ppo_hparams *hp, double *stats,
@@ -1101,7 +1236,8 @@
 
 static int launch_grad(const pfa_experience *exp, int64_t batch_rows, int32_t mb, const float *params,
                        const pfa_mlp_dims *dims, const pfa_ppo_hparams *hp, const double *adv_stats,
-                       int64_t global_mb_rows, float *grads, void *workspace, pfa_stream_t stream, int *grid_out) {
+                       int64_t global_mb_rows, float *grads, void *workspace, pfa_stream_t stream, int *grid_out,
+                       const int *sparse = nullptr ) {
     if (int rc = check_update_args(exp, batch_rows, dims, hp)) return rc;
     PFA_REQUIRE(dims && dims->hidden == kHidden, "ppo.grad: hidden must be %d", kHidden);
     PFA_REQUIRE(dims->obs_stride == 16 || dims->obs_stride == 32 || dims->obs_stride == 64 || dims->obs_stride == 96 ||
@@ -1151,25 +1287,27 @@
     }
     const int grid = grad_grid(mbs, dims->obs_stride);
 #define PFA_LAUNCH_GRAD_FULL(DPV, KKUV, MHV, KTMV, COLV) PFA_LAUNCH_GRAD_PERM(DPV, KKUV, MHV, KTMV, COLV, false)
-#define PFA_LAUNCH_GRAD_PERM(DPV, KKUV, MHV, KTMV, COLV, PERMV)                                                             \
+#define PFA_LAUNCH_GRAD_PERM(DPV, KKUV, MHV, KTMV, COLV, PERMV) PFA_LAUNCH_GRAD_FORM(DPV, KKUV, MHV, KTMV, COLV, PERMV, false)
+#define PFA_LAUNCH_GRAD_FORM(DPV, KKUV, MHV, KTMV, COLV, PERMV, GATHERV)                                                    \
     {                                                                                                                      \
         constexpr size_t lds_bytes = (size_t)GradLds<DPV, grad_glds(DPV, KTMV)>::kFloats * sizeof(float);                       \
         static_assert((size_t)2 * NativeLayout<DPV, KTMV, COLV>::kCount * sizeof(float) <= lds_bytes,                       \
                       "the two reduction buffers must fit in the tile/table area");                                       \
         static bool attr_set = false;                                                                                      \
         if (!attr_set) {                                                                                                   \
-            PFA_CHECK_HIP(hipFuncSetAttribute((const void *)ppo_mlp_grad_kernel<DPV, 0, KKUV, MHV, KTMV, COLV, PERMV>,     \
+            PFA_CHECK_HIP(hipFuncSetAttribute((const void *)ppo_mlp_grad_kernel<DPV, 0, KKUV, MHV, KTMV, COLV, PERMV, GATHERV>, \
                                               hipFuncAttributeMaxDynamicSharedMemorySize, (int)lds_bytes));                \
             attr_set = true;                                                                                               \
         }                                                                                                                  \
         if (grad_timed)                                                                                                    \
-            hipExtLaunchKernelGGL((ppo_mlp_grad_kernel<DPV, 0, KKUV, MHV, KTMV, COLV, PERMV>), dim3(grid), dim3(grad_threads(DPV)), \
-                                  lds_bytes, (hipStream_t)stream, grad_ev0, grad_ev1, 0, *exp, map, (long long)mbs, params,  \
-                                  dims->num_actions, dims->heads, *hp, adv_stats, (double)global_mb_rows, partials);      \
+            hipExtLaunchKernelGGL((ppo_mlp_grad_kernel<DPV, 0, KKUV, MHV, KTMV, COLV, PERMV, GATHERV>), dim3(grid), dim3(grad_threads(DPV)), \
+                                  lds_bytes, (hipStream_t)stream, both && !GATHERV ? nullptr : grad_ev0, both && GATHERV ? nullptr : grad_ev1, 0, *exp, map, \
+                                  (long long)mbs, params, dims->num_actions, dims->heads, *hp, adv_stats, (double)global_mb_rows, partials, \
+                                  sparse);                                                                                 \
         else                                                                                                               \
-            hipLaunchKernelGGL((ppo_mlp_grad_kernel<DPV, 0, KKUV, MHV, KTMV, COLV, PERMV>), dim3(grid), dim3(grad_threads(DPV)), \
+            hipLaunchKernelGGL((ppo_mlp_grad_kernel<DPV, 0, KKUV, MHV, KTMV, COLV, PERMV, GATHERV>), dim3(grid), dim3(grad_threads(DPV)), \
                                lds_bytes, (hipStream_t)stream, *exp, map, (long long)mbs, params, dims->num_actions,       \
-                               dims->heads, *hp, adv_stats, (double)global_mb_rows, partials);                             \
+                               dims->heads, *hp, adv_stats, (double)global_mb_rows, partials, sparse);                     \
     }
 #define PFA_LAUNCH_GRAD_KM(DPV, KKUV, MHV) PFA_LAUNCH_GRAD_FULL(DPV, KKUV, MHV, DPV / 16, false)
 #define PFA_LAUNCH_GRAD_K(DPV, KKUV) PFA_LAUNCH_GRAD_KM(DPV, KKUV, false)
@@ -1180,12 +1318,17 @@
         hipEvent_t grad_ev0 = nullptr, grad_ev1 = nullptr;
         const bool grad_timed = timing_pair("ppo_mlp_grad", &grad_ev0, &grad_ev1);
         ScopedKernelTimer timer(timing_ext_mode() ? nullptr : "ppo_mlp_grad", (hipStream_t)stream);
+        const bool both = grad_trimmed(dims) && sparse;
         switch (dims->obs_stride) {
             case 16: PFA_LAUNCH_GRAD(16) break;
             case 32: PFA_LAUNCH_GRAD(32) break;
             case 96: PFA_LAUNCH_GRAD(96) break;
             case 128: PFA_LAUNCH_GRAD(128) break;
             default:
+                if (both) {
+                    if (grad_perm(dims)) PFA_LAUNCH_GRAD_FORM(64, 13, false, 3, true, true, true)
+                    else PFA_LAUNCH_GRAD_FORM(64, 13, false, 3, true, false, true)
+                }
                 if (grad_trimmed(dims) && grad_perm(dims)) PFA_LAUNCH_GRAD_PERM(64, 13, false, 3, true, true)
                 else if (grad_trimmed(dims)) PFA_LAUNCH_GRAD_FULL(64, 13, false, 3, true)
                 else if (!dims->heads && (dims->obs_dim + 3) / 4 == 13) PFA_LAUNCH_GRAD_K(64, 13)
@@ -1196,6 +1339,7 @@
 #undef PFA_LAUNCH_GRAD_KM
 #undef PFA_LAUNCH_GRAD_FULL
 #undef PFA_LAUNCH_GRAD_PERM
+#undef PFA_LAUNCH_GRAD_FORM
 #undef PFA_LAUNCH_GRAD
 #undef PFA_LAUNCH_GRAD_K
     PFA_LAUNCH_CHECK();
@@ -1203,11 +1347,11 @@
     return 0;
 }
 
-extern "C" int pfa_ppo_mlp_grad(const pfa_experience *exp, int64_t batch_rows, int32_t mb, const float *params,
-                                const pfa_mlp_dims *dims, const pfa_ppo_hparams *hp, const double *adv_stats,
-                                int64_t global_mb_rows, float *grads, void *workspace, pfa_stream_t stream) {
+static int grad_and_reduce(const pfa_experience *exp, int64_t batch_rows, int32_t mb, const float *params,
+                           const pfa_mlp_dims *dims, const pfa_ppo_hparams *hp, const double *adv_stats,
+                           int64_t global_mb_rows, float *grads, void *workspace, pfa_stream_t stream, const int *sparse) {
     int grid = 0;
-    if (int rc = launch_grad(exp, batch_rows, mb, params, dims, hp, adv_stats, global_mb_rows, grads, workspace, stream, &grid)) return rc;
+    if (int rc = launch_grad(exp, batch_rows, mb, params, dims, hp, adv_stats, global_mb_rows, grads, workspace, stream, &grid, sparse)) return rc;
     float *partials = (float *)workspace;
     double *normp = norm_partials_of(workspace, dims);
     ScopedKernelTimer timer2("ppo_reduce", (hipStream_t)stream);
@@ -1230,6 +1374,12 @@
 #undef PFA_LAUNCH_REDUCE_P
     PFA_LAUNCH_CHECK();
     return 0;
+}
+
+extern "C" int pfa_ppo_mlp_grad(const pfa_experience *exp, int64_t batch_rows, int32_t mb, const float *params,
+                                const pfa_mlp_dims *dims, const pfa_ppo_hparams *hp, const double *adv_stats,
+                                int64_t global_mb_rows, float *grads, void *workspace, pfa_stream_t stream) {
+    return grad_and_reduce(exp, batch_rows, mb, params, dims, hp, adv_stats, global_mb_rows, grads, workspace, stream, nullptr);
 }
 
 extern "C" int pfa_ppo_mlp_grad_path(const pfa_mlp_dims *dims, int64_t mb_rows) { return dims && grad_bf16(dims, mb_rows) ? 1 : 0; }
@@ -1430,11 +1580,25 @@
     const bool fused = env_on("PFA_FUSED_ADAM", true) && reduce_adam_coresident(dims, fused_dp_wanted);
     const bool fused_dp = fused && fused_dp_wanted;
     const bool one_launch = fused && (!data_parallel || fused_dp);
+    int *sparse = nullptr;
+    if (dims && workspace && grad_trimmed(dims) && update_epochs > 0) {
+        int *word = (int *)((char *)workspace + sparse_offset(dims, hp->num_minibatches));
+        const bool scan = env_on("PFA_SPARSE_OBS", true) && update_epochs >= kSparseMinEpochs && exp->obs && pfa_igemm_get_products() != 1;
+        PFA_CHECK_HIP(hipMemsetAsync(word, scan ? 0 : 0xFF, sizeof(int), (hipStream_t)stream));
+        if (scan) {
+            sparse = word;
+            ScopedKernelTimer timer("obs_sparse_scan", (hipStream_t)stream);
+            hipLaunchKernelGGL(obs_sparse_scan_kernel, dim3((unsigned)((batch_rows + kScanBlockRows - 1) / kScanBlockRows)), dim3(kScanThreads), 0,
+                               (hipStream_t)stream, exp->obs, (long long)batch_rows, dims->obs_dim,
+                               reinterpret_cast<ObsCode *>(sparse + kSparseHeaderInts), sparse);
+            PFA_LAUNCH_CHECK();
+        }
+    }
     for (int e = 0; e < update_epochs; ++e)
         for (int mb = 0; mb < hp->num_minibatches; ++mb) {
             if (one_launch) {
                 int grid = 0;
-                if (int rc = launch_grad(exp, batch_rows, mb, params, dims, hp, adv_stats, global_mbs, grads, workspace, stream, &grid)) return rc;
+                if (int rc = launch_grad(exp, batch_rows, mb, params, dims, hp, adv_stats, global_mbs, grads, workspace, stream, &grid, sparse)) return rc;
                 ++opt_step;
                 LlArgs ll{};
                 if (fused_dp) ll = p2p_ll_next();
@@ -1446,7 +1610,7 @@
                 if (last && log_packed) *log_packed = 1;
                 continue;
             }
-            if (int rc = pfa_ppo_mlp_grad(exp, batch_rows, mb, params, dims, hp, adv_stats, global_mbs, grads, workspace, stream))
+            if (int rc = grad_and_reduce(exp, batch_rows, mb, params, dims, hp, adv_stats, global_mbs, grads, workspace, stream, sparse))
                 return rc;
             ++opt_step;
             if (data_parallel) {
@@ -1490,7 +1654,7 @@
         PFA_CHECK_HIP(hipFuncSetAttribute((const void *)ppo_mlp_grad_kernel<64, A, 13, false, 3, true>,                                \
                                           hipFuncAttributeMaxDynamicSharedMemorySize, (int)lds_bytes));                \
         hipLaunchKernelGGL((ppo_mlp_grad_kernel<64, A, 13, false, 3, true>), dim3(grid), dim3(grad_threads(64)), lds_bytes, (hipStream_t)stream, \
-                           *exp, map, (long long)mbs, params, dims->num_actions, 0u, *hp, adv_stats, (double)mbs, partials); \
+                           *exp, map, (long long)mbs, params, dims->num_actions, 0u, *hp, adv_stats, (double)mbs, partials, (const int *)nullptr); \
         break;
     switch (abl) {
         PFA_PROBE_CASE(0) PFA_PROBE_CASE(1) PFA_PROBE_CASE(2) PFA_PROBE_CASE(4) PFA_PROBE_CASE(6) PFA_PROBE_CASE(7)
```
